# mlelarge/graph_neural_net

Hardware: AMD Instinct MI355X
Metric: graph-pairs/sec FGNN fwd+bwd, N=50 regular pairs (higher is better)
Workload: dtype f32

## Files before the change

### graph_neural_net_amd/_lib.py

```python
import ctypes as C
import os

import torch

_HERE = os.path.dirname(os.path.abspath(__file__))
LIB_PATH = os.environ.get('FGNN_LIB') or os.path.join(_HERE, 'libfgnn_hip.so')

FGNN_H = 32
FGNN_TILE = 32
FGNN_MAX_DEPTH = 3
FGNN_RANGE_WG = 256
FGNN_LSAP_MAX_N = 2048
FGNN_SCORE_SPLIT = 4

c_float_p = C.c_void_p


class Slab(C.Structure):
    _fields_ = [('ptr', C.c_void_p), ('gstride', C.c_longlong), ('ldp', C.c_longlong), ('C', C.c_int),
                ('nrm', C.c_void_p), ('beta', C.c_void_p)]


class MlpFwdArgs(C.Structure):
    _fields_ = [('G', C.c_int), ('N', C.c_int), ('depth', C.c_int), ('nmlp', C.c_int),
                ('nvalid', C.c_void_p),
                ('a', Slab), ('b', Slab),
                ('W', (C.c_void_p * FGNN_MAX_DEPTH) * 2),
                ('bias', (C.c_void_p * FGNN_MAX_DEPTH) * 2),
                ('z', C.c_void_p * 2),
                ('ldz', C.c_longlong),
                ('part', C.c_void_p * 2),
                ('cnt', C.c_void_p), ('packed', C.c_void_p), ('xbits', C.c_void_p), ('xdeg', C.c_void_p),
                ('ranges', C.c_void_p), ('cu_share', C.c_int)]


class DwJob(C.Structure):
    _fields_ = [('dy', C.c_void_p), ('d_gstride', C.c_longlong), ('d_ld', C.c_longlong), ('relu_mask', C.c_void_p),
                ('x', C.c_void_p), ('x_gstride', C.c_longlong), ('x_ld', C.c_longlong), ('M', C.c_int), ('K', C.c_int)]


class ChainLayer(C.Structure):
    _fields_ = [('W', C.c_void_p), ('w_ostride', C.c_longlong), ('w_kstride', C.c_longlong), ('bias', C.c_void_p),
                ('M', C.c_int), ('K', C.c_int), ('relu', C.c_int), ('mask', C.c_void_p), ('out', C.c_void_p),
                ('o_gstride', C.c_longlong)]


class ChainArgs(C.Structure):
    _fields_ = [('x', C.c_void_p), ('x_gstride', C.c_longlong), ('x_ld', C.c_longlong), ('depth', C.c_int),
                ('layer', ChainLayer * 3), ('o_ld', C.c_longlong), ('nvalid', C.c_void_p), ('G', C.c_int), ('N', C.c_int)]


class Mlp64Args(C.Structure):
    _fields_ = [('x', C.c_void_p), ('x_gstride', C.c_longlong), ('x_ld', C.c_longlong), ('cin', C.c_int),
                ('xb', C.c_void_p), ('xb_gstride', C.c_longlong), ('xb_ld', C.c_longlong), ('cb', C.c_int),
                ('packed', C.c_void_p), ('nvalid', C.c_void_p), ('G', C.c_int), ('N', C.c_int),
                ('out', C.c_void_p), ('o_gstride', C.c_longlong), ('o_ld', C.c_longlong),
                ('dz', C.c_void_p), ('dz_gstride', C.c_longlong), ('dz_ld', C.c_longlong),
                ('dx', C.c_void_p), ('dx_gstride', C.c_longlong), ('dx_ld', C.c_longlong),
                ('dxb', C.c_void_p), ('dxb_gstride', C.c_longlong), ('dxb_ld', C.c_longlong),
                ('accumulate_dx', C.c_int), ('accumulate_dxb', C.c_int),
                ('wpart', C.c_void_p)]


class Mlp64PackJob(C.Structure):
    _fields_ = [('W', C.c_void_p * 3), ('bias', C.c_void_p * 3), ('cin', C.c_int), ('packed', C.c_void_p)]


class MlpBwdArgs(C.Structure):
    _fields_ = [('G', C.c_int), ('N', C.c_int), ('depth', C.c_int),
                ('nvalid', C.c_void_p),
                ('a', Slab), ('b', Slab),
                ('W', C.c_void_p * FGNN_MAX_DEPTH),
                ('bias', C.c_void_p * FGNN_MAX_DEPTH),
                ('dy', C.c_void_p), ('dgstride', C.c_longlong), ('ldd', C.c_longlong),
                ('z', C.c_void_p), ('zgstride', C.c_longlong), ('ldz', C.c_longlong),
                ('coef', C.c_void_p), ('s12', C.c_void_p), ('znrm', C.c_void_p),
                ('dxa', C.c_void_p), ('dxa_gstride', C.c_longlong), ('dxa_ld', C.c_longlong),
                ('dxb', C.c_void_p), ('dxb_gstride', C.c_longlong), ('dxb_ld', C.c_longlong),
                ('accumulate_a', C.c_int), ('accumulate_b', C.c_int),
                ('wpart', C.c_void_p), ('s12part', C.c_void_p), ('packed', C.c_void_p),
                ('s12tiles', C.c_void_p), ('s12_out', C.c_void_p), ('xbits', C.c_void_p), ('xdeg', C.c_void_p),
                ('ranges', C.c_void_p), ('cu_share', C.c_int)]


class Slab16(C.Structure):
    _fields_ = [('ptr', C.c_void_p), ('gstride', C.c_longlong), ('ldp', C.c_longlong), ('C', C.c_int),
                ('nrm', C.c_void_p), ('beta', C.c_void_p)]


class MlpFwd16Args(C.Structure):
    _fields_ = [('G', C.c_int), ('N', C.c_int), ('ldr', C.c_int), ('depth', C.c_int), ('nmlp', C.c_int),
                ('nvalid', C.c_void_p),
                ('a', Slab16), ('b', Slab16),
                ('z', C.c_void_p * 2), ('ldz', C.c_longlong),
                ('part', C.c_void_p * 2), ('cnt', C.c_void_p), ('packed', C.c_void_p), ('ranges', C.c_void_p)]


class MlpBwd16Args(C.Structure):
    _fields_ = [('G', C.c_int), ('N', C.c_int), ('ldr', C.c_int), ('depth', C.c_int),
                ('nvalid', C.c_void_p),
                ('a', Slab16), ('b', Slab16),
                ('dy', C.c_void_p), ('dgstride', C.c_longlong), ('ldd', C.c_longlong),
                ('z', C.c_void_p), ('zgstride', C.c_longlong), ('ldz', C.c_longlong),
                ('coef', C.c_void_p),
                ('dxa', C.c_void_p), ('dxa_gstride', C.c_longlong), ('dxa_ld', C.c_longlong),
                ('dxb', C.c_void_p), ('dxb_gstride', C.c_longlong), ('dxb_ld', C.c_longlong),
                ('accumulate_a', C.c_int), ('accumulate_b', C.c_int),
                ('wpart', C.c_void_p), ('s12part', C.c_void_p), ('packed', C.c_void_p), ('ranges', C.c_void_p)]


class GradJob(C.Structure):
    _fields_ = [('wpart', C.c_void_p), ('count', C.c_int), ('out', C.c_void_p), ('s12', C.c_void_p),
                ('nrm', C.c_void_p), ('dgn_w', C.c_void_p), ('dgn_b', C.c_void_p), ('rows', C.c_int), ('scale', C.c_float), ('scale_dev', C.c_void_p)]


class PackJob(C.Structure):
    _fields_ = [('kind', C.c_int), ('ca', C.c_int), ('cb', C.c_int), ('depth', C.c_int), ('nmlp', C.c_int),
                ('W', (C.c_void_p * FGNN_MAX_DEPTH) * 2), ('bias', (C.c_void_p * FGNN_MAX_DEPTH) * 2),
                ('out', C.c_void_p)]


class PairgenArgs(C.Structure):
    _fields_ = [('seed', C.c_ulonglong), ('first', C.c_longlong), ('B', C.c_int), ('N', C.c_int),
                ('family', C.c_int), ('noise_model', C.c_int), ('edge_density', C.c_double),
                ('thr_edge', C.c_ulonglong), ('thr_noise1', C.c_ulonglong), ('thr_noise2', C.c_ulonglong),
                ('thr_vertex', C.c_ulonglong), ('swaps_per_edge', C.c_int),
                ('bits1', C.c_void_p), ('bits2', C.c_void_p), ('nvalid', C.c_void_p)]


MAX_GRAD_JOBS = 16
MAX_PACK_JOBS = 24
_VP, _LL, _I, _F = C.c_void_p, C.c_longlong, C.c_int, C.c_float

_SIGNATURES = {
    'fgnn_last_error': [],
    'fgnn_version': [],
    'fgnn_tiles_per_graph': [_I],
    'fgnn_mlp_bwd_num_workgroups': [],
    'fgnn_pack_floats': [_I, _I, _I, _I, _I],
    'fgnn_pack_operands': [_VP, _I, _VP],
    'fgnn_mlp_fwd': [C.POINTER(MlpFwdArgs), _VP],
    'fgnn_pack_x3_floats': [_I, _I, _I, _I, _I],
    'fgnn_pack_x3_operands': [_VP, _I, _VP],
    'fgnn_mlp_fwd_x3': [C.POINTER(MlpFwdArgs), _VP],
    'fgnn_debug_mlp_fwd_masks': [C.POINTER(MlpFwdArgs), _VP, _VP, _VP],
    'fgnn_debug_mlp_fwd_x3_masks': [C.POINTER(MlpFwdArgs), _VP, _VP, _VP],
    'fgnn_debug_matmul_variant': [_I],
    'fgnn_gn_finalize': [_VP, _VP, _VP, _VP, _I, _I, _I, _F, _VP, _VP],
    'fgnn_gn_finalize2': [_VP, _VP, _VP, _VP, _VP, _VP, _I, _I, _I, _F, _VP, _VP, _VP],
    'fgnn_gn_plane_supported': [_I],
    'fgnn_gn_plane_fwd': [_VP, _LL, _LL, _VP, _VP, _VP, _I, _I, _I, _F, _VP, _LL, _LL, _VP, _VP],
    'fgnn_gn_plane_bwd': [_VP, _LL, _LL, _VP, _LL, _LL, _VP, _VP, _I, _I, _I, _VP, _LL, _LL, _VP, _VP, _VP, _VP],
    'fgnn_gn_stats': [_VP, _LL, _LL, _VP, _VP, _I, _I, _I, _F, _VP, _VP],
    'fgnn_gn_apply': [_VP, _LL, _LL, _VP, _VP, _VP, _I, _I, _I, _VP, _LL, _LL, _VP],
    'fgnn_ragged_tile_ranges': [_VP, _I, _I, _VP, _VP],
    'fgnn_ragged_tile_ranges_order': [_VP, _I, _I, _VP, _VP, _VP],
    'fgnn_ragged_tile_ranges16': [_VP, _I, _I, _I, _VP, _VP],
    'fgnn_conv1x1_dw_multi': [C.POINTER(DwJob), _I, _VP, _I, _I, _VP, _VP],
    'fgnn_conv_chain_supported': [_I, _I, C.POINTER(C.c_int)],
    'fgnn_conv_chain': [C.POINTER(ChainArgs), _VP],
    'fgnn_mlp64_supported': [_I, _I, _I],
    'fgnn_mlp64_num_workgroups': [],
    'fgnn_mlp64_param_count': [_I],
    'fgnn_mlp64_packed_floats': [_I],
    'fgnn_mlp64_pack': [_VP, _VP, _VP, _VP, _VP, _VP, _I, _VP, _VP],
    'fgnn_mlp64_pack_multi': [C.POINTER(Mlp64PackJob), _I, _VP],
    'fgnn_mlp64_fwd': [C.POINTER(Mlp64Args), _VP],
    'fgnn_mlp64_bwd': [C.POINTER(Mlp64Args), _VP],
    'fgnn_conv1x1': [_VP, _LL, _LL, _VP, _VP, _LL, _LL, _VP, _I, _VP, _I, _I, _I, _I, _VP, _LL, _LL, _VP],
    'fgnn_conv1x1_dw_chunks': [_I, _I],
    'fgnn_conv1x1_dw': [_VP, _LL, _LL, _VP, _VP, _LL, _LL, _VP, _I, _I, _I, _I, _VP, _VP],
    'fgnn_chan_matmul_fwd': [C.POINTER(Slab), C.POINTER(Slab), _VP, _I, _I, _VP, _LL, _LL, _VP],
    'fgnn_chan_matmul_fwd_ord': [C.POINTER(Slab), C.POINTER(Slab), _VP, _I, _I, _VP, _LL, _LL, _VP, _I, _VP],
    'fgnn_chan_matmul_fwd_fin_supported': [_I],
    'fgnn_chan_matmul_fwd_fin': [C.POINTER(Slab), C.POINTER(Slab), _VP, _VP, _VP, _VP, _VP, _F, _VP, _I, _I, _VP, _LL, _LL, _VP],
    'fgnn_chan_matmul_fwd_fin_ord': [C.POINTER(Slab), C.POINTER(Slab), _VP, _VP, _VP, _VP, _VP, _F, _VP, _I, _I, _VP, _LL, _LL, _VP, _I, _VP],
    'fgnn_colmax_fwd': [C.POINTER(Slab), _VP, _I, _I, _VP, _VP, _VP],
    'fgnn_colmax_fwd_fin_supported': [_I],
    'fgnn_colmax_fwd_fin': [C.POINTER(Slab), _VP, _VP, _VP, _F, _VP, _I, _I, _VP, _VP, _VP],
    'fgnn_score_ce_fwd': [_VP, _VP, _VP, _I, _I, _I, _VP, _VP, _VP, _VP],
    'fgnn_score_row_blocks': [_I, _I],
    'fgnn_score_ce_fwd_blocks': [_VP, _VP, _VP, _I, _I, _I, _I, _VP, _VP, _VP, _VP],
    'fgnn_score_ce_bwd': [_VP, _VP, _VP, _VP, _VP, _VP, _I, _I, _I, _VP, _VP, _VP],
    'fgnn_inv_node_count': [_VP, _I, _VP, _VP],
    'fgnn_score_bwd': [_VP, _VP, _VP, _VP, _I, _I, _I, _VP, _VP, _VP],
    'fgnn_ce_fwd': [_VP, _VP, _I, _I, _VP, _VP, _VP],
    'fgnn_ce_bwd': [_VP, _VP, _VP, _VP, _I, _I, _VP, _VP],
    'fgnn_colmax_bwd': [_VP, _VP, _VP, _I, _I, _I, _VP, _LL, _LL, C.POINTER(Slab), _VP, _VP],
    'fgnn_gn_bwd_stats': [_VP, _LL, _LL, _VP, _LL, _LL, _VP, _VP, _I, _I, _I, _VP, _VP],
    'fgnn_gn_bwd_coef': [_VP, _VP, _VP, _I, _I, _I, _VP, _VP, _VP, _VP],
    'fgnn_gn_bwd_coef_tiles': [_VP, _VP, _VP, _I, _I, _I, _VP, _VP, _VP],
    'fgnn_grad_finalize': [_VP, _I, _I, _I, _I, _VP],
    'fgnn_gn_bwd_apply': [_VP, _LL, _LL, _VP, _LL, _LL, _VP, _VP, _I, _I, _I, _VP, _LL, _LL, _VP],
    'fgnn_mlp_bwd': [C.POINTER(MlpBwdArgs), _VP],
    'fgnn_mlp_bwd_x3': [C.POINTER(MlpBwdArgs), _VP],
    'fgnn_mlp_bwd_pair': [C.POINTER(MlpBwdArgs), C.POINTER(MlpBwdArgs), _VP],
    'fgnn_mlp_bwd_t16': [C.POINTER(MlpBwdArgs), _VP],
    'fgnn_mlp_bwd_t16_supported': [C.POINTER(MlpBwdArgs)],
    'fgnn_mlp_bwd_pair_t16': [C.POINTER(MlpBwdArgs), C.POINTER(MlpBwdArgs), _VP],
    'fgnn_mlp_bwd_pair_x3': [C.POINTER(MlpBwdArgs), C.POINTER(MlpBwdArgs), _VP],
    'fgnn_block1_struct_supported': [_I, _I, _I],
    'fgnn_block1_struct_table_floats': [_I],
    'fgnn_block1_struct_ws_floats': [_I, _I],
    'fgnn_block1_struct_rows': [_I, _I],
    'fgnn_block1_struct_fwd': [_VP, _VP, _I, _I, _VP, _VP, _VP, _VP, _VP, C.c_float, _VP, _VP, _VP, _LL, _LL, _VP, _VP, _VP, _VP, _VP, _VP, _VP],
    'fgnn_block1_struct_bwd': [_VP, _VP, _I, _I, _VP, _VP, _VP, _VP, _VP, _VP, _VP, _VP, _LL, _LL, _VP, _VP, _VP, _VP, _VP, _VP],
    'fgnn_block1_struct_fwd_pack': [_VP, _VP, _I, _I, _VP, _VP, _VP, _VP, _VP, C.c_float, _VP, _VP, _VP, _LL, _LL, _VP, _VP, _VP, _VP, _VP, _VP, _VP, _I, _VP],
    'fgnn_block1_struct_fwd16_pack': [_VP, _VP, _I, _I, _I, _VP, _VP, _VP, _VP, _VP, C.c_float, _VP, _VP, _VP, _LL, _LL, _VP, _VP, _VP, _VP, _VP, _VP, _VP, _I, _VP],
    'fgnn_block1_struct_fwd16': [_VP, _VP, _I, _I, _I, _VP, _VP, _VP, _VP, _VP, C.c_float, _VP, _VP, _VP, _LL, _LL, _VP, _VP, _VP, _VP, _VP, _VP, _VP],
    'fgnn_block1_struct_bwd16': [_VP, _VP, _I, _I, _I, _VP, _VP, _VP, _VP, _VP, _VP, _VP, _VP, _LL, _LL, _VP, _VP, _VP, _VP, _VP, _VP],
    'fgnn_mlp_bwd_coef_tiles_supported': [_I, _I],
    'fgnn_mlp_param_count': [_I, _I],
    'fgnn_reduce_partials': [_VP, _I, _I, _VP, _VP],
    'fgnn_chan_matmul_bwd': [C.POINTER(Slab), C.POINTER(Slab), _VP, _LL, _LL, _VP, _I, _I, _VP, _VP, _LL, _LL, _VP, _VP, _VP],
    'fgnn_chan_matmul_bwd_ord': [C.POINTER(Slab), C.POINTER(Slab), _VP, _LL, _LL, _VP, _I, _I, _VP, _VP, _LL, _LL, _VP, _VP, _VP, _I, _VP],
    'fgnn_sum_scale': [_VP, _I, _I, _F, _VP, _VP],
    'fgnn_adam_step': [_VP, _VP, _VP, _VP, _I, C.c_double, C.c_double, C.c_double, C.c_double, _I, C.c_double, _VP],
    'fgnn_adam_step_dev': [_VP, _VP, _VP, _VP, _I, _VP, _VP, _VP],
    'fgnn_expand_adjacency': [_VP, _VP, _I, _I, _VP, _VP],
    'fgnn_pack_adjacency': [_VP, _VP, _I, _I, _VP, _VP, _VP],
    'fgnn_pack_adjacency_ld': [_VP, _VP, _I, _I, _I, _VP, _VP, _VP],
    'fgnn_pack_adjacency_pair': [_VP, _VP, _VP, _VP, _I, _I, _I, _VP, _VP, _VP, _VP, _VP],
    'fgnn_adjacency_degree': [_VP, _VP, _I, _I, _VP, _VP],
    'fgnn_accuracy_max': [_VP, _VP, _I, _I, _VP, _VP],
    'fgnn_lsap_accuracy': [_VP, _LL, _I, _VP, _I, _I, _VP, _VP, _VP],
    'fgnn_pairgen_supported': [_I, _I, _I],
    'fgnn_pairgen': [C.POINTER(PairgenArgs), _VP],
    'fgnn_tiles_per_graph16': [_I, _I],
    'fgnn_to_bf16': [_VP, _VP, _I, _I, _I, _I, _VP, _LL, _LL, _VP],
    'fgnn_from_bf16': [_VP, _LL, _LL, _I, _I, _I, _I, _VP, _VP],
    'fgnn_pack16_floats': [_I, _I, _I, _I, _I],
    'fgnn_pack16_operands': [_VP, _I, _VP],
    'fgnn_mlp_fwd16': [C.POINTER(MlpFwd16Args), _VP],
    'fgnn_debug_mlp_fwd16_masks': [C.POINTER(MlpFwd16Args), _VP, _VP, _VP],
    'fgnn_gn_finalize_tpg': [_VP, _VP, _VP, _VP, _I, _I, _I, _I, _F, _VP, _VP],
    'fgnn_gn_finalize2_tpg': [_VP, _VP, _VP, _VP, _VP, _VP, _I, _I, _I, _I, _F, _VP, _VP, _VP],
    'fgnn_gn_bwd_coef_tiles_tpg': [_VP, _VP, _VP, _I, _I, _I, _I, _VP, _VP, _VP],
    'fgnn_chan_matmul_fwd16': [C.POINTER(Slab16), C.POINTER(Slab16), _VP, _I, _I, _I, _VP, _LL, _LL, _VP],
    'fgnn_chan_matmul_fwd16_fin': [C.POINTER(Slab16), C.POINTER(Slab16), _VP, _VP, _VP, _VP, _VP, _F, _I, _VP, _I, _I, _I, _VP, _LL,
                                   _LL, _VP],
    'fgnn_chan_matmul_bwd16': [C.POINTER(Slab16), C.POINTER(Slab16), _VP, _LL, _LL, _VP, _I, _I, _I, _VP, _VP, _LL, _LL, _VP, _VP, _VP],
    'fgnn_chan_matmul_bwd16_t': [C.POINTER(Slab16), C.POINTER(Slab16), _VP, _LL, _LL, _VP, _I, _VP, _I, _I, _I, _VP, _VP, _LL, _LL,
                                 _VP, _VP, _VP],
    'fgnn_chan_matmul_bwd16_tc': [C.POINTER(Slab16), C.POINTER(Slab16), _VP, _LL, _LL, _VP, _I, _VP, _I, _I, _I, _VP, _VP, _LL, _LL,
                                  _VP, _VP, _VP, _VP, _VP],
    'fgnn_colmax_bwd16_coef': [_VP, _VP, _VP, _I, _I, _I, _I, _VP, _LL, _LL, C.POINTER(Slab16), _VP, _VP, _VP],
    'fgnn_colmax_fwd16': [C.POINTER(Slab16), _VP, _I, _I, _I, _VP, _VP, _VP],
    'fgnn_colmax_bwd16': [_VP, _VP, _VP, _I, _I, _I, _I, _VP, _LL, _LL, C.POINTER(Slab16), _VP, _VP],
    'fgnn_mlp_bwd16': [C.POINTER(MlpBwd16Args), _VP],
    'fgnn_mlp_bwd16_pair': [C.POINTER(MlpBwd16Args), C.POINTER(MlpBwd16Args), _VP],
}
_RESTYPES = {'fgnn_last_error': C.c_char_p, 'fgnn_block1_struct_ws_floats': C.c_longlong}
EXPORTS = tuple(_SIGNATURES)

_lib = None


def load():
    global _lib
    if _lib is not None:
        return _lib
    if not os.path.exists(LIB_PATH):
        raise RuntimeError(
            'graph_neural_net_amd: %s is missing. Build it with '
            '`python -c "import __graft_entry__ as g; g.build()"` or `make -C graph_neural_net_amd/csrc`. '
            'There is no CPU fallback.' % LIB_PATH)
    lib = C.CDLL(LIB_PATH)
    for name, argtypes in _SIGNATURES.items():
        fn = getattr(lib, name)
        fn.argtypes = argtypes
        fn.restype = _RESTYPES.get(name, C.c_int)
# ... 73 lines not shown
```

### graph_neural_net_amd/csrc/mlp_bwd.hip

```cpp
#include "fgnn_common.h"
#include "fgnn_pack.h"

#ifdef FGNN_PHASES
__device__ unsigned long long *g_phase_buf = nullptr;
__device__ int g_phase_sel = 0;
#define PH_DECL unsigned long long ph_[16] = {0, 0, 0, 0, 0, 0, 0, 0, 0, 0, 0, 0, 0, 0, 0, 0}; unsigned long long ph_last_ = __builtin_amdgcn_s_memtime();
#define PH(k) { const unsigned long long t_ = __builtin_amdgcn_s_memtime(); ph_[k] += t_ - ph_last_; ph_last_ = t_; }
#define PH_FLUSH if (g_phase_buf && g_phase_sel == CA * 100 + CB && (threadIdx.x & 63) == 0) { for (int k_ = 0; k_ < 16; ++k_) g_phase_buf[((long long)blockIdx.x * NW + wv) * 16 + k_] = ph_[k_]; }
#else
#define PH_DECL
#define PH(k) __builtin_amdgcn_sched_barrier(0);
#define PH_FLUSH
#endif

namespace {

constexpr int TLD = 36;
constexpr int TILE_F = 32 * TLD;
constexpr int BWD_WG = 256;

struct TileCtx {
    int g, tt, p, i, jj;
    bool inb;
};
// ... 628 lines not shown
    static_assert(PCOUNT % 4 == 0, "partials are summed four at a time");
    float4 *out = reinterpret_cast<float4 *>(A.wpart + (long long)blockIdx.x * PCOUNT);
    const float4 *part4 = reinterpret_cast<const float4 *>(smem);
    for (int e = threadIdx.x; e < PCOUNT / 4; e += 64 * NW) {
        float4 a = part4[e];
#pragma unroll
        for (int w = 1; w < NW; ++w) {
            const float4 b = part4[w * (PCOUNT / 4) + e];
            a.x += b.x;
            a.y += b.y;
            a.z += b.z;
            a.w += b.w;
        }
        out[e] = a;
    }
    PH(11)
    PH_FLUSH
}

template <int CA, int CB, int DEPTH, bool PK = false, bool SKIP = false>
int launch_bwd_impl(const fgnn_mlp_bwd_args *a, int tpg, int total, hipStream_t st) {
    constexpr int LDS = BwdLayout<CA, CB, DEPTH>::LDS_F * 4;
    static_assert(LDS <= 160 * 1024, "LDS budget");
    static LdsAttrCache attr_cache;
    (void)fgnn_raise_lds(attr_cache, (const void *)mlp_bwd_kernel<CA, CB, DEPTH, PK, SKIP>, LDS);
    hipLaunchKernelGGL((mlp_bwd_kernel<CA, CB, DEPTH, PK, SKIP>), dim3(a->cu_share == 2 && !SKIP ? BWD_WG / 2 : BWD_WG), dim3(64 * NW), LDS, st,
                       *a, tpg, total);
    FGNN_LAUNCH_CHECK();
    return 0;
}
template <int CA, int CB, int DEPTH, bool PK = false>
int launch_bwd(const fgnn_mlp_bwd_args *a, int tpg, int total, hipStream_t st) {
    static_assert(BWD_WG == FGNN_RANGE_WG, "fgnn_ragged_tile_ranges splits for the backward grid");
    if (a->ranges) return launch_bwd_impl<CA, CB, DEPTH, PK, true>(a, tpg, total, st);
    return launch_bwd_impl<CA, CB, DEPTH, PK, false>(a, tpg, total, st);
}

template <int DEPTH>
int dispatch_c(const fgnn_mlp_bwd_args *a, int tpg, int total, hipStream_t st) {
    const int ca = a->a.C, cb = a->b.C;
    if (a->xbits) {
        if constexpr (DEPTH == 3) {
            if (ca == 2 && cb == 0) return launch_bwd<2, 0, DEPTH, true>(a, tpg, total, st);
            if (ca == 32 && cb == 2) return launch_bwd<32, 2, DEPTH, true>(a, tpg, total, st);
        }
        fgnn_set_error("fgnn_mlp_bwd: xbits needs depth 3 and a 2-channel slab (2 or 32+2 input channels), got depth %d, %d + %d",
                       DEPTH, ca, cb);
        return 1;
    }
#define FGNN_CASE(A_, B_) \
    if (ca == A_ && cb == B_) return launch_bwd<A_, B_, DEPTH>(a, tpg, total, st);
    FGNN_CASE(2, 0)
    FGNN_CASE(16, 0)
    FGNN_CASE(32, 0)
    FGNN_CASE(32, 2)
    FGNN_CASE(32, 32)
#undef FGNN_CASE
    fgnn_set_error("fgnn_mlp_bwd: unsupported input channels (%d + %d); built for 2, 16, 32, 32+2, 32+32", ca, cb);
    return 1;
}

}

#ifdef FGNN_PHASES
extern "C" int fgnn_debug_phase_buffer(void *p, int ca, int cb) {
    const int sel = ca * 100 + cb;
    if (hipMemcpyToSymbol(HIP_SYMBOL(g_phase_sel), &sel, sizeof(sel)) != hipSuccess) return 1;
    return hipMemcpyToSymbol(HIP_SYMBOL(g_phase_buf), &p, sizeof(p)) == hipSuccess ? 0 : 1;
}
#endif

extern "C" int fgnn_mlp_bwd_num_workgroups(void) { return BWD_WG; }

extern "C" int fgnn_mlp_bwd_coef_tiles_supported(int G, int N) {
    const long long tpg = fgnn_tiles_per_graph(N), total = (long long)G * tpg;
    const long long per_wg = (total + BWD_WG - 1) / BWD_WG;
    return (per_wg + tpg - 2) / tpg + 1 <= FGNN_BWD_COEF_GRAPHS ? 1 : 0;
}

extern "C" int fgnn_mlp_param_count(int Cin, int depth) { return 32 * Cin + 32 + (depth - 1) * (32 * 32 + 32); }

extern "C" int fgnn_mlp_bwd(const fgnn_mlp_bwd_args *a, void *stream) {
    FGNN_CHECK(a != nullptr, "fgnn_mlp_bwd: null args");
    FGNN_CHECK(a->G > 0 && a->N > 0, "fgnn_mlp_bwd: bad G=%d N=%d", a->G, a->N);
    FGNN_CHECK(a->depth >= 1 && a->depth <= FGNN_MAX_DEPTH, "fgnn_mlp_bwd: depth %d not in 1..%d", a->depth, FGNN_MAX_DEPTH);
    const bool pk_a = a->xbits && a->a.C == 2, pk_b = a->xbits && a->b.C == 2;
    FGNN_CHECK((a->a.ptr || pk_a) && a->a.C > 0, "fgnn_mlp_bwd: slab a missing");
    FGNN_CHECK(a->b.C == 0 || a->b.ptr || pk_b, "fgnn_mlp_bwd: slab b has channels but no pointer");
    FGNN_CHECK(!a->xbits || a->xdeg, "fgnn_mlp_bwd: xbits without xdeg (fgnn_adjacency_degree)");
    FGNN_CHECK(!(pk_a && a->dxa) && !(pk_b && a->dxb), "fgnn_mlp_bwd: no gradient with respect to the packed adjacency");
    FGNN_CHECK(a->dy && a->z && a->wpart, "fgnn_mlp_bwd: missing dy/z/wpart");
    FGNN_CHECK(a->coef || (a->s12 && a->znrm) || (a->s12tiles && a->znrm), "fgnn_mlp_bwd: need coef, or s12 + znrm, or s12tiles + znrm");
    {
        const long long lim = 0x7fffffffll / 4, G = a->G;
        FGNN_CHECK(G * a->a.gstride < lim && G * a->b.gstride < lim && G * a->dgstride < lim && G * a->zgstride < lim &&
                   G * a->dxa_gstride < lim && G * a->dxb_gstride < lim,
                   "fgnn_mlp_bwd: a tensor exceeds 2 GiB (32-bit buffer addressing); split the batch");
    }
    for (int l = 0; l < a->depth; ++l) FGNN_CHECK(a->W[l] && a->bias[l], "fgnn_mlp_bwd: missing weights layer %d", l);
    const int tpg = fgnn_tiles_per_graph(a->N);
    const long long total = (long long)a->G * tpg;
    FGNN_CHECK(total < (1ll << 30), "fgnn_mlp_bwd: too many tiles");
    FGNN_CHECK(!a->ranges || (a->nvalid && !a->s12tiles), "fgnn_mlp_bwd: ranges need nvalid and exclude s12tiles");
    FGNN_CHECK(!a->s12tiles || a->b.C > 0, "fgnn_mlp_bwd: s12tiles is built into the two-slab kernels only; use fgnn_gn_bwd_coef_tiles");
    FGNN_CHECK(!a->s12tiles || fgnn_mlp_bwd_coef_tiles_supported(a->G, a->N),
               "fgnn_mlp_bwd: s12tiles needs a workgroup's tile range to span <= %d graphs (G=%d N=%d); "
               "use fgnn_gn_bwd_coef_tiles", FGNN_BWD_COEF_GRAPHS, a->G, a->N);
    hipStream_t st = (hipStream_t)stream;
    if (a->depth == 1) return dispatch_c<1>(a, tpg, (int)total, st);
    if (a->depth == 2) return dispatch_c<2>(a, tpg, (int)total, st);
    return dispatch_c<3>(a, tpg, (int)total, st);
}
```

### graph_neural_net_amd/csrc/mlp_bwd_pair.hip

```cpp
#include "fgnn_tile.h"
#include "fgnn_pack.h"

namespace {

constexpr int BWD_WG = 256;
constexpr int NW = 8;
constexpr int NP = 4;

DEVI float4 coef_from_sums(const float4 n, const float2 sv, float nv) {
    const float m = nv * nv;
    float4 k;
    k.x = n.x;
    k.y = n.y;
    k.z = m > 0.f ? -n.y * sv.y * n.w / m : 0.f;
    k.w = m > 0.f ? -n.y * sv.x / m : 0.f;
    return k;
}
DEVI float4 coef_record(const fgnn_mlp_bwd_args &A, int g, int ch) {
    if (A.coef) return reinterpret_cast<const float4 *>(A.coef)[(long long)g * FGNN_H + ch];
    const float4 n = reinterpret_cast<const float4 *>(A.znrm)[(long long)g * FGNN_H + ch];
    const float2 sv = reinterpret_cast<const float2 *>(A.s12)[(long long)g * FGNN_H + ch];
    return coef_from_sums(n, sv, (float)nvalid_of(A.nvalid, g, A.N));
}

// ... 360 lines not shown
        }
    }

    constexpr int PCOUNT = L::PCOUNT;
#pragma unroll
    for (int l = 0; l < DEPTH; ++l) db[l] += __shfl_xor(db[l], 32);
    if constexpr (VW0) {
#pragma unroll
        for (int r = 0; r < 32; ++r) w0v[r] = half_sum(w0v[r]);
#pragma unroll
        for (int r = 0; r < 16; ++r) b0v[r] = half_sum(b0v[r]);
    }
    __syncthreads();
    {
        float *red = smem + wv * PCOUNT;
#pragma unroll
        for (int r = 0; r < 16; ++r) {
            const int o = ch_of(r, h);
            if constexpr (VW0) {
                if (j == 0) {
                    red[o * CA] = w0v[2 * r];
                    red[o * CA + 1] = w0v[2 * r + 1];
                    red[32 * CA + o] = b0v[r];
                }
            } else {
                if (j < CA) red[o * CA + j] = dW0a[r];
            }
        }
        int off = 32 * CA;
#pragma unroll
        for (int l = 0; l < DEPTH; ++l) {
            if (l > 0) {
#pragma unroll
                for (int r = 0; r < 16; ++r) red[off + ch_of(r, h) * 32 + j] = dWh[l - 1][r];
                off += 1024;
            }
            if (h == 0 && !(VW0 && l == 0)) red[off + j] = db[l];
            off += 32;
        }
    }
    __syncthreads();
    static_assert(PCOUNT % 4 == 0, "partials are summed four at a time");
    const float4 *part4 = reinterpret_cast<const float4 *>(smem);
    for (int e = threadIdx.x; e < 2 * (PCOUNT / 4); e += 64 * NW) {
        const int m = e >= PCOUNT / 4 ? 1 : 0, ee = e - m * (PCOUNT / 4);
        float4 a = part4[(4 * m) * (PCOUNT / 4) + ee];
#pragma unroll
        for (int w = 1; w < NP; ++w) {
            const float4 b = part4[(4 * m + w) * (PCOUNT / 4) + ee];
            a.x += b.x;
            a.y += b.y;
            a.z += b.z;
            a.w += b.w;
        }
        reinterpret_cast<float4 *>(P.m[m].wpart + (long long)blockIdx.x * PCOUNT)[ee] = a;
    }
}

template <int CA, bool PK, bool SKIP>
int launch_pair_impl(const fgnn_mlp_bwd_args *a1, const fgnn_mlp_bwd_args *a2, int tpg, int total, hipStream_t st) {
    constexpr int LDS = PairLayout<CA>::LDS_F * 4;
    static_assert(LDS <= 160 * 1024, "LDS budget");
    static LdsAttrCache attr_cache;
    (void)fgnn_raise_lds(attr_cache, (const void *)mlp_bwd_pair_kernel<CA, PK, SKIP>, LDS);
    PairArgs P;
    P.m[0] = *a1;
    P.m[1] = *a2;
    hipLaunchKernelGGL((mlp_bwd_pair_kernel<CA, PK, SKIP>), dim3(a1->cu_share == 2 && !SKIP ? BWD_WG / 2 : BWD_WG), dim3(64 * NW), LDS, st, P,
                       tpg, total);
    FGNN_LAUNCH_CHECK();
    return 0;
}
template <int CA, bool PK>
int launch_pair(const fgnn_mlp_bwd_args *a1, const fgnn_mlp_bwd_args *a2, int tpg, int total, hipStream_t st) {
    static_assert(BWD_WG == FGNN_RANGE_WG, "fgnn_ragged_tile_ranges splits for the backward grid");
    if (a1->ranges) return launch_pair_impl<CA, PK, true>(a1, a2, tpg, total, st);
    return launch_pair_impl<CA, PK, false>(a1, a2, tpg, total, st);
}

}

extern "C" int fgnn_mlp_bwd_pair(const fgnn_mlp_bwd_args *a1, const fgnn_mlp_bwd_args *a2, void *stream) {
    FGNN_CHECK(a1 && a2, "fgnn_mlp_bwd_pair: null args");
    FGNN_CHECK(BWD_WG == fgnn_mlp_bwd_num_workgroups(), "fgnn_mlp_bwd_pair: workgroup count differs from fgnn_mlp_bwd");
    FGNN_CHECK(a1->G > 0 && a1->N > 0 && a1->G == a2->G && a1->N == a2->N && a1->depth == a2->depth,
               "fgnn_mlp_bwd_pair: the two MLPs must share G, N and depth");
    FGNN_CHECK(mlp_bwd_pair_supported(a1->a.C, a1->depth) && a1->b.C == 0 && a2->b.C == 0,
               "fgnn_mlp_bwd_pair: built for depth 3 and ONE input slab of 2 or 32 channels (got depth %d, %d + %d); use fgnn_mlp_bwd",
               a1->depth, a1->a.C, a1->b.C);
    FGNN_CHECK(a1->a.ptr == a2->a.ptr && a1->a.C == a2->a.C && a1->a.gstride == a2->a.gstride && a1->a.ldp == a2->a.ldp &&
               a1->a.nrm == a2->a.nrm && a1->a.beta == a2->a.beta && a1->xbits == a2->xbits && a1->xdeg == a2->xdeg &&
               a1->nvalid == a2->nvalid, "fgnn_mlp_bwd_pair: the two MLPs must read the same input slab");
    FGNN_CHECK(a1->ranges == a2->ranges && (!a1->ranges || a1->nvalid), "fgnn_mlp_bwd_pair: both MLPs take the same ranges (with nvalid)");
    FGNN_CHECK(a1->packed && a2->packed, "fgnn_mlp_bwd_pair: needs both operand images (fgnn_pack_operands, kind 1)");
    FGNN_CHECK(!a1->dxa && !a1->s12part, "fgnn_mlp_bwd_pair: the input gradient and its tile sums belong to the SECOND argument block");
    FGNN_CHECK(!a1->s12tiles && !a2->s12tiles, "fgnn_mlp_bwd_pair: s12tiles is an mlp3 feature");
    const bool pk_a = a1->xbits && a1->a.C == 2;
    FGNN_CHECK((a1->a.ptr || pk_a), "fgnn_mlp_bwd_pair: slab a missing");
    FGNN_CHECK(!a1->xbits || a1->xdeg, "fgnn_mlp_bwd_pair: xbits without xdeg (fgnn_adjacency_degree)");
    FGNN_CHECK(!(a2->dxa && a2->a.C != 32), "fgnn_mlp_bwd_pair: the input gradient exists for the 32-channel slab only; use fgnn_mlp_bwd");
    for (const fgnn_mlp_bwd_args *a : {a1, a2}) {
        FGNN_CHECK(a->dy && a->z && a->wpart, "fgnn_mlp_bwd_pair: missing dy/z/wpart");
        FGNN_CHECK(a->coef || (a->s12 && a->znrm), "fgnn_mlp_bwd_pair: need coef, or s12 + znrm");
        const long long lim = 0x7fffffffll / 4, G = a->G;
        FGNN_CHECK(G * a->a.gstride < lim && G * a->dgstride < lim && G * a->zgstride < lim && G * a->dxa_gstride < lim,
                   "fgnn_mlp_bwd_pair: a tensor exceeds 2 GiB (32-bit buffer addressing); split the batch");
    }
    const int tpg = fgnn_tiles_per_graph(a1->N);
    const long long total = (long long)a1->G * tpg;
    FGNN_CHECK(total < (1ll << 30), "fgnn_mlp_bwd_pair: too many tiles");
    hipStream_t st = (hipStream_t)stream;
    if (a1->xbits) return launch_pair<2, true>(a1, a2, tpg, (int)total, st);
    if (a1->a.C == 2) return launch_pair<2, false>(a1, a2, tpg, (int)total, st);
    return launch_pair<32, false>(a1, a2, tpg, (int)total, st);
}
```

### graph_neural_net_amd/csrc/mlp_bwd_pair_t16.hip

```cpp
#include "fgnn_t16.h"
#include "fgnn_pack.h"

#ifdef FGNN_PHASES
__device__ unsigned long long *g_phase16_buf = nullptr;
#define PH_DECL unsigned long long ph_[16] = {0, 0, 0, 0, 0, 0, 0, 0, 0, 0, 0, 0, 0, 0, 0, 0}; unsigned long long ph_last_ = __builtin_amdgcn_s_memtime();
#define PH(k) { const unsigned long long t_ = __builtin_amdgcn_s_memtime(); ph_[k] += t_ - ph_last_; ph_last_ = t_; }
#define PH_FLUSH if (g_phase16_buf && (threadIdx.x & 63) == 0) { for (int k_ = 0; k_ < 16; ++k_) g_phase16_buf[((long long)blockIdx.x * NW + wv) * 16 + k_] = ph_[k_]; }
#else
#define PH_DECL
#define PH(k)
#define PH_FLUSH
#endif

namespace {

using namespace t16;

constexpr int BWD_WG = 256;
constexpr int NW = 8;
constexpr int NP = 4;

DEVI float4 coef_from_sums(const float4 n, const float2 sv, float nv) {
    const float m = nv * nv;
    float4 k;
// ... 336 lines not shown
    if constexpr (SKIP) {
        if (emit) {
            for (int t = T0 + pair; t < T1; t += NP) {
                const int g = t / tpg, tt = t - g * tpg;
                if (tile_live(tt, A.N, A.nvalid[g])) continue;
                if (lane < 32) reinterpret_cast<float2 *>(P.m[1].s12part)[((long long)g * tpg + tt) * FGNN_H + lane] = make_float2(0.f, 0.f);
            }
        }
    }

    constexpr int PCOUNT = L::PCOUNT;
#pragma unroll
    for (int b = 0; b < 2; ++b) {
        db0[b] += __shfl_xor(db0[b], 16);
        db0[b] += __shfl_xor(db0[b], 32);
        db1[b] += __shfl_xor(db1[b], 16);
        db1[b] += __shfl_xor(db1[b], 32);
        db2[b] += __shfl_xor(db2[b], 16);
        db2[b] += __shfl_xor(db2[b], 32);
    }
    __syncthreads();
    PH(10)
    {
        float *red = smem + wv * PCOUNT;
        auto put = [&](int off, const f32x4 (&dW)[4], const float (&db)[2]) {
#pragma unroll
            for (int mb = 0; mb < 2; ++mb)
#pragma unroll
                for (int nb = 0; nb < 2; ++nb)
#pragma unroll
                    for (int r = 0; r < 4; ++r) red[off + row_chan(16 * mb + 4 * q + r) * 32 + row_chan(16 * nb + px)] = dW[2 * mb + nb][r];
            if (q == 0) {
                red[off + 1024 + row_chan(px)] = db[0];
                red[off + 1024 + row_chan(16 + px)] = db[1];
            }
        };
        put(0, dW0, db0);
        put(1056, dW1, db1);
        put(2112, dW2, db2);
    }
    __syncthreads();
    static_assert(PCOUNT % 4 == 0 && PCOUNT == 3 * 1056, "partials are summed four at a time");
    const float4 *part4 = reinterpret_cast<const float4 *>(smem);
    for (int e = threadIdx.x; e < 2 * (PCOUNT / 4); e += 64 * NW) {
        const int m = e >= PCOUNT / 4 ? 1 : 0, ee = e - m * (PCOUNT / 4);
        float4 a = part4[(4 * m) * (PCOUNT / 4) + ee];
#pragma unroll
        for (int w = 1; w < NP; ++w) {
            const float4 b = part4[(4 * m + w) * (PCOUNT / 4) + ee];
            a.x += b.x;
            a.y += b.y;
            a.z += b.z;
            a.w += b.w;
        }
        reinterpret_cast<float4 *>(P.m[m].wpart + (long long)blockIdx.x * PCOUNT)[ee] = a;
    }
    PH(11)
    PH_FLUSH
}

template <bool SKIP, bool HAS_DX>
int launch_pair16(const fgnn_mlp_bwd_args *a1, const fgnn_mlp_bwd_args *a2, int tpg, int total, hipStream_t st) {
    constexpr int LDS = PairLayout16::LDS_F * 4;
    static_assert(LDS <= 160 * 1024, "LDS budget");
    static LdsAttrCache attr_cache;
    (void)fgnn_raise_lds(attr_cache, (const void *)mlp_bwd_pair_t16_kernel<SKIP, HAS_DX>, LDS);
    PairArgs P;
    P.m[0] = *a1;
    P.m[1] = *a2;
    hipLaunchKernelGGL((mlp_bwd_pair_t16_kernel<SKIP, HAS_DX>), dim3(a1->cu_share == 2 && !SKIP ? BWD_WG / 2 : BWD_WG), dim3(64 * NW), LDS, st, P, tpg,
                       total);
    FGNN_LAUNCH_CHECK();
    return 0;
}

}

#ifdef FGNN_PHASES
extern "C" int fgnn_debug_phase_buffer_t16(void *p) { return hipMemcpyToSymbol(HIP_SYMBOL(g_phase16_buf), &p, sizeof(p)) == hipSuccess ? 0 : 1; }
#endif

extern "C" int fgnn_mlp_bwd_pair_t16(const fgnn_mlp_bwd_args *a1, const fgnn_mlp_bwd_args *a2, void *stream) {
    FGNN_CHECK(a1 && a2, "fgnn_mlp_bwd_pair_t16: null args");
    FGNN_CHECK(BWD_WG == fgnn_mlp_bwd_num_workgroups() && BWD_WG == FGNN_RANGE_WG, "fgnn_mlp_bwd_pair_t16: workgroup count differs from fgnn_mlp_bwd");
    FGNN_CHECK(a1->G > 0 && a1->N > 0 && a1->G == a2->G && a1->N == a2->N && a1->depth == a2->depth,
               "fgnn_mlp_bwd_pair_t16: the two MLPs must share G, N and depth");
    FGNN_CHECK(a1->depth == 3 && a1->a.C == 32 && a1->b.C == 0 && a2->b.C == 0 && !a1->xbits && !a2->xbits,
               "fgnn_mlp_bwd_pair_t16: built for depth 3 and ONE dense input slab of 32 channels (got depth %d, %d + %d); use fgnn_mlp_bwd_pair",
               a1->depth, a1->a.C, a1->b.C);
    FGNN_CHECK(a1->a.ptr && a1->a.ptr == a2->a.ptr && a1->a.C == a2->a.C && a1->a.gstride == a2->a.gstride && a1->a.ldp == a2->a.ldp &&
               a1->a.nrm == a2->a.nrm && a1->a.beta == a2->a.beta && a1->nvalid == a2->nvalid,
               "fgnn_mlp_bwd_pair_t16: the two MLPs must read the same input slab");
    FGNN_CHECK(a1->ranges == a2->ranges && (!a1->ranges || a1->nvalid), "fgnn_mlp_bwd_pair_t16: both MLPs take the same ranges (with nvalid)");
    FGNN_CHECK(a1->packed && a2->packed, "fgnn_mlp_bwd_pair_t16: needs both operand images (fgnn_pack_operands, kind 5)");
    FGNN_CHECK(!a1->dxa && !a1->s12part, "fgnn_mlp_bwd_pair_t16: the input gradient and its tile sums belong to the SECOND argument block");
    FGNN_CHECK(!a1->s12tiles && !a2->s12tiles, "fgnn_mlp_bwd_pair_t16: s12tiles is an mlp3 feature");
    FGNN_CHECK(a1->N <= 256, "fgnn_mlp_bwd_pair_t16: N <= 256 (division-free pixel decode)");
    for (const fgnn_mlp_bwd_args *a : {a1, a2}) {
        FGNN_CHECK(a->dy && a->z && a->wpart, "fgnn_mlp_bwd_pair_t16: missing dy/z/wpart");
        FGNN_CHECK(a->coef || (a->s12 && a->znrm), "fgnn_mlp_bwd_pair_t16: need coef, or s12 + znrm");
        const long long lim = 0x7fffffffll / 4, G = a->G;
        FGNN_CHECK(G * a->a.gstride < lim && G * a->dgstride < lim && G * a->zgstride < lim && G * a->dxa_gstride < lim,
                   "fgnn_mlp_bwd_pair_t16: a tensor exceeds 2 GiB (32-bit buffer addressing); split the batch");
    }
    const int tpg = fgnn_tiles_per_graph(a1->N);
    const long long total = (long long)a1->G * tpg;
    FGNN_CHECK(total < (1ll << 29), "fgnn_mlp_bwd_pair_t16: too many tiles");
    hipStream_t st = (hipStream_t)stream;
    if (a2->dxa) return a1->ranges ? launch_pair16<true, true>(a1, a2, tpg, (int)total, st) : launch_pair16<false, true>(a1, a2, tpg, (int)total, st);
    return a1->ranges ? launch_pair16<true, false>(a1, a2, tpg, (int)total, st) : launch_pair16<false, false>(a1, a2, tpg, (int)total, st);
}
```

### graph_neural_net_amd/csrc/mlp_bwd_pair_x3.hip

```cpp
#include "fgnn_tile.h"
#include "fgnn_pack.h"
#include "fgnn_x3.h"

namespace {

#ifdef FGNN_PHASES
__device__ unsigned long long *g_px3_phase_buf = nullptr;
#define PH_DECL unsigned long long ph_[16] = {0, 0, 0, 0, 0, 0, 0, 0, 0, 0, 0, 0, 0, 0, 0, 0}; unsigned long long ph_last_ = __builtin_amdgcn_s_memtime();
#define PH(k) { const unsigned long long t_ = __builtin_amdgcn_s_memtime(); ph_[k] += t_ - ph_last_; ph_last_ = t_; }
#define PH_FLUSH if (g_px3_phase_buf && CA == 32 && (threadIdx.x & 63) == 0) { for (int k_ = 0; k_ < 16; ++k_) g_px3_phase_buf[((long long)blockIdx.x * NW + wv) * 16 + k_] = ph_[k_]; }
#else
#define PH_DECL
#define PH(k)
#define PH_FLUSH
#endif

constexpr int BWD_WG = 256;
constexpr int NW = 8;
constexpr int NP = 4;

DEVI float4 coef_from_sums(const float4 n, const float2 sv, float nv) {
    const float m = nv * nv;
    float4 k;
    k.x = n.x;
// ... 359 lines not shown
        prev_tile = tile;
        PH(8)
    }

    constexpr int PCOUNT = L::PCOUNT;
    float db[DEPTH];
#pragma unroll
    for (int l = 0; l < DEPTH; ++l) {
        db[l] = -ndb[l];
        db[l] += __shfl_xor(db[l], 32);
    }
    f32x16 dWh[2];
#pragma unroll
    for (int r = 0; r < 16; ++r) {
        dWh[0][r] = PARK[r * 64 + lane];
        dWh[1][r] = PARK[1024 + r * 64 + lane];
    }
    PH(12)
    __syncthreads();
    PH(10)
    {
        float *red = smem + wv * PCOUNT;
#pragma unroll
        for (int r = 0; r < 16; ++r) {
            const int o = ch_of(r, h);
            if (j < CA) red[o * CA + j] = dW0a[r];
        }
        int off = 32 * CA;
#pragma unroll
        for (int l = 0; l < DEPTH; ++l) {
            if (l > 0) {
#pragma unroll
                for (int r = 0; r < 16; ++r) red[off + ch_of(r, h) * 32 + j] = dWh[l - 1][r];
                off += 1024;
            }
            if (h == 0) red[off + j] = db[l];
            off += 32;
        }
    }
    __syncthreads();
    static_assert(PCOUNT % 4 == 0, "partials are summed four at a time");
    const float4 *part4 = reinterpret_cast<const float4 *>(smem);
    for (int e = threadIdx.x; e < 2 * (PCOUNT / 4); e += 64 * NW) {
        const int m = e >= PCOUNT / 4 ? 1 : 0, ee = e - m * (PCOUNT / 4);
        float4 a = part4[(4 * m) * (PCOUNT / 4) + ee];
#pragma unroll
        for (int w = 1; w < NP; ++w) {
            const float4 b = part4[(4 * m + w) * (PCOUNT / 4) + ee];
            a.x += b.x;
            a.y += b.y;
            a.z += b.z;
            a.w += b.w;
        }
        reinterpret_cast<float4 *>(P.m[m].wpart + (long long)blockIdx.x * PCOUNT)[ee] = a;
    }
    PH(11)
    PH_FLUSH
}

template <int CA, bool PK>
int launch_pair_x3(const fgnn_mlp_bwd_args *a1, const fgnn_mlp_bwd_args *a2, int tpg, int total, hipStream_t st) {
    constexpr int LDS = PairX3Layout<CA>::LDS_F * 4;
    static_assert(LDS <= 160 * 1024, "LDS budget");
    static LdsAttrCache attr_cache;
    (void)fgnn_raise_lds(attr_cache, (const void *)mlp_bwd_pair_x3_kernel<CA, PK>, LDS);
    PairArgs P;
    P.m[0] = *a1;
    P.m[1] = *a2;
    hipLaunchKernelGGL((mlp_bwd_pair_x3_kernel<CA, PK>), dim3(a1->cu_share == 2 ? BWD_WG / 2 : BWD_WG), dim3(64 * NW), LDS, st, P, tpg, total);
    FGNN_LAUNCH_CHECK();
    return 0;
}

}

#ifdef FGNN_PHASES
extern "C" int fgnn_debug_phase_buffer_px3(void *p) {
    return hipMemcpyToSymbol(HIP_SYMBOL(g_px3_phase_buf), &p, sizeof(p)) == hipSuccess ? 0 : 1;
}
#endif

extern "C" int fgnn_mlp_bwd_pair_x3(const fgnn_mlp_bwd_args *a1, const fgnn_mlp_bwd_args *a2, void *stream) {
    FGNN_CHECK(a1 && a2, "fgnn_mlp_bwd_pair_x3: null args");
    FGNN_CHECK(BWD_WG == fgnn_mlp_bwd_num_workgroups(), "fgnn_mlp_bwd_pair_x3: workgroup count differs from fgnn_mlp_bwd");
    FGNN_CHECK(a1->G > 0 && a1->N > 0 && a1->G == a2->G && a1->N == a2->N && a1->depth == a2->depth,
               "fgnn_mlp_bwd_pair_x3: the two MLPs must share G, N and depth");
    FGNN_CHECK(mlp_bwd_pair_supported(a1->a.C, a1->depth) && a1->b.C == 0 && a2->b.C == 0,
               "fgnn_mlp_bwd_pair_x3: built for depth 3 and ONE input slab of 2 or 32 channels (got depth %d, %d + %d); use fgnn_mlp_bwd",
               a1->depth, a1->a.C, a1->b.C);
    FGNN_CHECK(a1->a.ptr == a2->a.ptr && a1->a.C == a2->a.C && a1->a.gstride == a2->a.gstride && a1->a.ldp == a2->a.ldp &&
               a1->a.nrm == a2->a.nrm && a1->a.beta == a2->a.beta && a1->xbits == a2->xbits && a1->xdeg == a2->xdeg &&
               a1->nvalid == a2->nvalid, "fgnn_mlp_bwd_pair_x3: the two MLPs must read the same input slab");
    FGNN_CHECK(!a1->ranges && !a2->ranges, "fgnn_mlp_bwd_pair_x3: no padding-tile skipping (ranges); use fgnn_mlp_bwd_pair for ragged batches");
    FGNN_CHECK(a1->packed && a2->packed, "fgnn_mlp_bwd_pair_x3: needs both operand images (fgnn_pack_x3_operands, kind 1)");
    FGNN_CHECK(!a1->dxa && !a1->s12part, "fgnn_mlp_bwd_pair_x3: the input gradient and its tile sums belong to the SECOND argument block");
    FGNN_CHECK(!a1->s12tiles && !a2->s12tiles, "fgnn_mlp_bwd_pair_x3: s12tiles is an mlp3 feature");
    const bool pk_a = a1->xbits && a1->a.C == 2;
    FGNN_CHECK((a1->a.ptr || pk_a), "fgnn_mlp_bwd_pair_x3: slab a missing");
    FGNN_CHECK(!a1->xbits || a1->xdeg, "fgnn_mlp_bwd_pair_x3: xbits without xdeg (fgnn_adjacency_degree)");
    FGNN_CHECK(!(a2->dxa && a2->a.C != 32), "fgnn_mlp_bwd_pair_x3: the input gradient exists for the 32-channel slab only; use fgnn_mlp_bwd");
    FGNN_CHECK(a1->ldd == a1->ldz && a2->ldd == a1->ldd && a2->ldz == a1->ldd && (!a2->dxa || a2->dxa_ld == a1->ldd) &&
               (a1->a.C != 32 || a1->a.ldp == a1->ldd),
               "fgnn_mlp_bwd_pair_x3: dy, z, d_in (and a 32-channel input slab) must share one channel stride");
    for (const fgnn_mlp_bwd_args *a : {a1, a2}) {
        FGNN_CHECK(a->dy && a->z && a->wpart, "fgnn_mlp_bwd_pair_x3: missing dy/z/wpart");
        FGNN_CHECK(a->coef || (a->s12 && a->znrm), "fgnn_mlp_bwd_pair_x3: need coef, or s12 + znrm");
        const long long lim = 0x7fffffffll / 4, G = a->G;
        FGNN_CHECK(G * a->a.gstride < lim && G * a->dgstride < lim && G * a->zgstride < lim && G * a->dxa_gstride < lim,
                   "fgnn_mlp_bwd_pair_x3: a tensor exceeds 2 GiB (32-bit buffer addressing); split the batch");
    }
    const int tpg = fgnn_tiles_per_graph(a1->N);
    const long long total = (long long)a1->G * tpg;
    FGNN_CHECK(total < (1ll << 30), "fgnn_mlp_bwd_pair_x3: too many tiles");
    hipStream_t st = (hipStream_t)stream;
    if (a1->xbits) return launch_pair_x3<2, true>(a1, a2, tpg, (int)total, st);
    if (a1->a.C == 2) return launch_pair_x3<2, false>(a1, a2, tpg, (int)total, st);
    return launch_pair_x3<32, false>(a1, a2, tpg, (int)total, st);
}
```

### graph_neural_net_amd/csrc/mlp_bwd_t16.hip

```cpp
#include "fgnn_t16.h"
#include "fgnn_pack.h"

namespace {

using namespace t16;

constexpr int BWD_WG = 256;
constexpr int NW = 8;

DEVI float4 coef_from_sums(const float4 n, const float2 sv, float nv) {
    const float m = nv * nv;
    float4 k;
    k.x = n.x;
    k.y = n.y;
    k.z = m > 0.f ? -n.y * sv.y * n.w / m : 0.f;
    k.w = m > 0.f ? -n.y * sv.x / m : 0.f;
    return k;
}
DEVI int graph_nv(const rsrc_t &rnv, bool ragged, int g, int N) {
    const int v = __builtin_amdgcn_raw_buffer_load_b32(rnv, g * 4, 0, 0);
    return __builtin_amdgcn_readfirstlane(ragged ? v : N);
}

template <int CB>
struct Layout16 {
    static constexpr int DEPTH = 3;
    static constexpr PkBwd PK = pk_bwd(32, CB, DEPTH);
    static constexpr int OFF_W0A = PK.off_w1a, OFF_W0B = PK.off_w1b, OFF_W1 = PK.off_wh, OFF_WT1 = PK.off_wt, OFF_WT2 = PK.off_wt + 16;
    static constexpr int OFF_WT0A = PK.off_wt0a, OFF_WT0B = PK.off_wt0b;
    static constexpr int BIAS_F = PK.bias_f;
    static constexpr int WEIGHT_F = pk_pad_floats(PK.floats);
    static constexpr int NSLOT = 5;
    static constexpr int CIN = 32 + CB;
    static constexpr int PCOUNT = 32 * CIN + 32 + (DEPTH - 1) * (32 * 32 + 32);
    static constexpr int TILE_OFF = WEIGHT_F;
    static constexpr int REC_OFF = TILE_OFF + NW * NSLOT * TILE_F;
    static constexpr int WGK_OFF = REC_OFF + NW * 256;
    static constexpr int LIVE_OFF = WGK_OFF + FGNN_BWD_COEF_GRAPHS * 128;
    static constexpr int MAIN_F = LIVE_OFF + LIVE_LIST_CAP + NW;
    static constexpr int RED_F = NW * PCOUNT;
    static constexpr int LDS_F = MAIN_F > RED_F ? MAIN_F : RED_F;
};

template <int CB, bool PKD, bool SKIP, bool DXB>
__global__ __launch_bounds__(64 * NW, 2) void mlp_bwd_t16_kernel(const fgnn_mlp_bwd_args A, const int tpg, const int total_tiles) {
    extern __shared__ __attribute__((aligned(16))) float smem[];
    using L = Layout16<CB>;
    constexpr bool NB = CB == 32;
    const int lane = threadIdx.x & 63, wv = __builtin_amdgcn_readfirstlane(threadIdx.x >> 6);
    const int px = lane & 15, q = lane >> 4;
    const int P2 = A.N * A.N, hpg = 2 * tpg;
    const View va = make_view(A.a.ptr, A.a.gstride, A.a.ldp, A.G);
    const View vb = make_view(A.b.ptr, A.b.gstride, A.b.ldp, A.G);
    PackedSrc ps = {};
    if constexpr (PKD) ps = make_packed_src(A.xbits, A.xdeg, A.G, A.N);
    const View vdy = make_view(A.dy, A.dgstride, A.ldd, A.G);
    const View vz = make_view(A.z, A.zgstride, A.ldz, A.G);
    const View vdxa = make_view(A.dxa, A.dxa_gstride, A.dxa_ld, A.G);
    const View vdxb = make_view(A.dxb, A.dxb_gstride, A.dxb_ld, A.G);

    float *wl = smem;
    float *my = smem + L::TILE_OFF + wv * (L::NSLOT * TILE_F);
    float *XA = my, *XB = my + TILE_F, *S0 = my + 2 * TILE_F, *S1 = my + 3 * TILE_F, *S2 = my + 4 * TILE_F;
    const int lane_base = tile_lane_base(px, q);

    f32x4 dW0a[4], dW0b[4], dW1[4], dW2[4];
    float db0[2] = {0.f, 0.f}, db1[2] = {0.f, 0.f}, db2[2] = {0.f, 0.f}, dbx[2] = {0.f, 0.f};
#pragma unroll
    for (int k = 0; k < 4; ++k) dW0a[k] = dW0b[k] = dW1[k] = dW2[k] = zero4();

    const int nwg = gridDim.x;
    const int qq = total_tiles / nwg, rem = total_tiles % nwg;
    int T0 = blockIdx.x * qq + ((int)blockIdx.x < rem ? (int)blockIdx.x : rem);
    int T1 = T0 + qq + ((int)blockIdx.x < rem ? 1 : 0);
    if constexpr (SKIP) {
        T0 = A.ranges[blockIdx.x];
        T1 = A.ranges[blockIdx.x + 1];
    }
    const int H0 = 2 * T0, H1 = 2 * T1;
    const bool ragged = A.nvalid != nullptr;
    const rsrc_t rnv = __builtin_amdgcn_make_buffer_rsrc(const_cast<int *>(A.nvalid), 0, ragged ? A.G * 4 : 0, 0x00020000);
    const float rcpN = 1.f / (float)A.N;
    const bool from_tiles = A.s12tiles != nullptr;
    const int g0 = T0 / tpg;
    float4 *wgK = reinterpret_cast<float4 *>(smem + L::WGK_OFF);

    int live_cnt = 0;
    int *live_list = reinterpret_cast<int *>(smem + L::LIVE_OFF);
    int nlive = 0, lk = wv - NW;
    bool use_list = false;
    if constexpr (SKIP) {
        nlive = build_live_list(live_list, live_list + LIVE_LIST_CAP, T0, T1, tpg, FGNN_TILE, A.N, A.nvalid, threadIdx.x, 64 * NW);
        use_list = nlive <= LIVE_LIST_CAP;
    }
    auto next_half = [&](int h) {
        if constexpr (SKIP) {
            if (use_list) {
                int r = H1;
                while (true) {
                    lk += NW;
                    if ((lk >> 1) >= nlive) break;
                    const int t = live_list[lk >> 1], g = t / tpg, hh = 2 * (t - g * tpg) + (lk & 1);
                    if (hh * 16 < P2) {
                        r = 2 * t + (lk & 1);
                        break;
                    }
                }
                return __builtin_amdgcn_readfirstlane(r);
            }
            while (h < H1) {
                const int g = h / hpg, hh = h - g * hpg;
                const int nv = A.nvalid[g];
                if (hh * 16 < P2 && tile_live(hh >> 1, A.N, nv)) {
                    const bool mine = live_cnt % NW == wv;
                    ++live_cnt;
                    if (mine) break;
                    ++h;
                } else if ((hh >> 1) * FGNN_TILE / A.N >= nv) {
                    h = (g + 1) * hpg;
                } else {
                    ++h;
                }
            }
            return __builtin_amdgcn_readfirstlane(h < H1 ? h : H1);
        } else {
            while (h < H1) {
                const int g = h / hpg, hh = h - g * hpg;
                if (hh * 16 < P2) break;
                h += NW;
            }
            return __builtin_amdgcn_readfirstlane(h);
        }
    };

    pk_glds<NW>(smem, A.packed, L::WEIGHT_F, wv, lane);

    float mean[8], av[8], beta[8], kx[8], ky[8], kz[8], kw[8];
#pragma unroll
    for (int s = 0; s < 8; ++s) {
        mean[s] = 0.f;
        av[s] = 1.f;
        beta[s] = (NB && A.b.nrm && A.b.beta) ? A.b.beta[chan_s(s) + chan_q(q)] : 0.f;
        kx[s] = ky[s] = kz[s] = kw[s] = 0.f;
    }
    float4 *rec = reinterpret_cast<float4 *>(smem + L::REC_OFF) + wv * 64;
    auto fetch_records = [&](int g, int nv) {
        if (lane < 32) {
            float4 k4;
            if (from_tiles) k4 = wgK[(g - g0) * 32 + lane];
            else if (A.coef) k4 = reinterpret_cast<const float4 *>(A.coef)[(long long)g * FGNN_H + lane];
            else {
                const float4 n = reinterpret_cast<const float4 *>(A.znrm)[(long long)g * FGNN_H + lane];
                const float2 sv = reinterpret_cast<const float2 *>(A.s12)[(long long)g * FGNN_H + lane];
                k4 = coef_from_sums(n, sv, (float)nv);
            }
            rec[lane] = k4;
            if (NB && A.b.nrm) rec[32 + lane] = reinterpret_cast<const float4 *>(A.b.nrm)[(long long)g * A.b.C + lane];
        }
    };
    auto read_records = [&]() {
#pragma unroll
        for (int s = 0; s < 8; ++s) {
            const float4 k4 = rec[chan_s(s) + chan_q(q)];
            kx[s] = k4.x;
            ky[s] = k4.y;
            kz[s] = k4.z;
            kw[s] = k4.w;
            if (NB && A.b.nrm) {
                const float4 n = rec[32 + chan_s(s) + chan_q(q)];
                mean[s] = n.x;
                av[s] = n.y;
            }
        }
    };

    constexpr int NXB = CB == 32 ? 8 : 1;
    float xa[8], xb[NXB], dyr[8], zr[8];
    auto load_x = [&](int h) {
        const bool act = h < H1;
        const int g = __builtin_amdgcn_readfirstlane(act ? h / hpg : 0);
        const int p = (act ? h - g * hpg : 0) * 16 + px;
        const bool inb = act && p < P2;
        load8(xa, va, lane_voff(va, q, p, inb), g * va.gs4);
        if constexpr (CB == 32) {
            load8(xb, vb, lane_voff(vb, q, p, inb), g * vb.gs4);
        } else if constexpr (PKD) {
            int i, jj;
            row_col(p, A.N, rcpN, i, jj);
            const int ob = (inb && q == 0) ? (i * ps.words + (jj >> 5)) * 4 : OOB_OFF;
            const int od = (inb && q == 1 && i == jj) ? i * 4 : OOB_OFF;
            const unsigned w = (unsigned)__builtin_amdgcn_raw_buffer_load_b32(ps.bits, ob, g * ps.N * ps.words * 4, 0);
            const float d = __builtin_bit_cast(float, __builtin_amdgcn_raw_buffer_load_b32(ps.deg, od, g * ps.N * 4, 0));
            xb[0] = q == 0 ? (((w >> (jj & 31)) & 1u) ? 1.f : 0.f) : d;
        } else {
            xb[0] = buf_load(vb, (inb && q < 2) ? q * vb.ld4 + 4 * p : OOB_OFF, g * vb.gs4);
        }
    };
    auto load_dyz = [&](int h) {
        const bool act = h < H1;
        const int g = __builtin_amdgcn_readfirstlane(act ? h / hpg : 0);
        const int p = (act ? h - g * hpg : 0) * 16 + px;
        const bool inb = act && p < P2;
        load8(dyr, vdy, lane_voff(vdy, q, p, inb), g * vdy.gs4);
        load8(zr, vz, lane_voff(vz, q, p, inb), g * vz.gs4);
    };

    int h = next_half(SKIP ? H0 : H0 + wv);
    load_x(h);
    int cached_g = -1, cur_nv = A.N;

    if (from_tiles) {
        const int g1 = T1 > T0 ? (T1 - 1) / tpg : g0 - 1;
        float2 *scr = reinterpret_cast<float2 *>(smem + L::TILE_OFF);
        const int cc = threadIdx.x & 31, sl = threadIdx.x >> 5;
        for (int g = g0; g <= g1; ++g) {
            float p1 = 0.f, p2 = 0.f;
            constexpr int TS = (64 * NW) / 32, U = 8;
            for (int t0 = sl; t0 < tpg; t0 += TS * U) {
                float2 v[U];
#pragma unroll
                for (int k = 0; k < U; ++k) {
                    const int t = t0 + TS * k;
                    v[k] = reinterpret_cast<const float2 *>(A.s12tiles)[((long long)g * tpg + (t < tpg ? t : 0)) * FGNN_H + cc];
                }
#pragma unroll
                for (int k = 0; k < U; ++k) {
                    if (t0 + TS * k < tpg) {
                        p1 += v[k].x;
                        p2 += v[k].y;
                    }
                }
            }
            scr[sl * 32 + cc] = make_float2(p1, p2);
            __syncthreads();
            if (threadIdx.x < 32) {
                float s1 = 0.f, s2 = 0.f;
#pragma unroll
                for (int k = 0; k < (64 * NW) / 32; ++k) {
                    s1 += scr[k * 32 + cc].x;
                    s2 += scr[k * 32 + cc].y;
                }
                const float2 sv = make_float2(s1, s2);
                if (A.s12_out) reinterpret_cast<float2 *>(A.s12_out)[(long long)g * FGNN_H + cc] = sv;
                const float4 n = reinterpret_cast<const float4 *>(A.znrm)[(long long)g * FGNN_H + cc];
                wgK[(g - g0) * 32 + cc] = coef_from_sums(n, sv, (float)graph_nv(rnv, ragged, g, A.N));
            }
            __syncthreads();
        }
    }
    if (h < H1) {
        const int g = h / hpg;
        cur_nv = graph_nv(rnv, ragged, g, A.N);
        fetch_records(g, cur_nv);
        cached_g = g;
    }
    if constexpr (CB == 2) {
        for (int e = lane; e < 16 * TLD; e += 64) XB[e] = 0.f;
    }
    __syncthreads();
    load_dyz(h);
    if (cached_g >= 0) read_records();

    while (h < H1) {
        const int hn = next_half(SKIP ? h + 1 : h + NW);
        const int g = __builtin_amdgcn_readfirstlane(h / hpg), hh = h - g * hpg;
        const int p = hh * 16 + px;
        const bool inb = p < P2;
        if (g != cached_g) {
            cur_nv = graph_nv(rnv, ragged, g, A.N);
            fetch_records(g, cur_nv);
            read_records();
            cached_g = g;
        }
        bool valid = inb;
        if (ragged) {
            int i, jj;
            row_col(p, A.N, rcpN, i, jj);
            valid = inb && i < cur_nv && jj < cur_nv;
        }
        const bool full = __ballot(valid) == ~0ull;

        float h1[8], h2[8];
        {
            float yb[NXB];
            if constexpr (NB) {
#pragma unroll
                for (int s = 0; s < 8; ++s) yb[s] = (xb[s] - mean[s]) * av[s] + beta[s];
            } else {
                yb[0] = xb[0];
            }
            stage8(XA, lane_base, xa);
            if constexpr (CB == 32) {
                stage8(XB, lane_base, yb);
            } else {
                if (q < 2) XB[8 * q * TLD + px] = yb[0];
            }
            f32x4 acc[2];
            load_bias(acc, wl + L::BIAS_F, 0, q);
            gemm32<L::OFF_W0A>(acc, wl, xa, lane);
            if constexpr (CB == 32) gemm32<L::OFF_W0B>(acc, wl, yb, lane);
            else gemm2<L::OFF_W0B>(acc, wl, q < 2 ? yb[0] : 0.f, lane);
            load_x(hn);
#pragma unroll
            for (int s = 0; s < 8; ++s) h1[s] = relu1(acc[s >> 2][s & 3]);
            stage8(S0, lane_base, h1);
            load_bias(acc, wl + L::BIAS_F, 1, q);
            gemm32<L::OFF_W1>(acc, wl, h1, lane);
#pragma unroll
            for (int s = 0; s < 8; ++s) h2[s] = relu1(acc[s >> 2][s & 3]);
            stage8(S1, lane_base, h2);
        }
        float dpre[8];
#pragma unroll
        for (int s = 0; s < 8; ++s) dpre[s] = fmaf(kz[s], zr[s] - kx[s], fmaf(ky[s], dyr[s], kw[s]));
        if (!full) {
#pragma unroll
            for (int s = 0; s < 8; ++s) dpre[s] = valid ? dpre[s] : 0.f;
        }
        stage8(S2, lane_base, dpre);
        load_dyz(hn);
        __builtin_amdgcn_sched_barrier(0);
        {
            f32x4 a2[2];
            a2[0] = a2[1] = zero4();
            gemm32<L::OFF_WT2>(a2, wl, dpre, lane);
            wgrad16(dW2, db2, S2, S1, lane);
#pragma unroll
            for (int s = 0; s < 8; ++s) dpre[s] = h2[s] > 0.f ? a2[s >> 2][s & 3] : 0.f;
        }
        __builtin_amdgcn_sched_barrier(0);
        stage8(S1, lane_base, dpre);
        {
            f32x4 a2[2];
            a2[0] = a2[1] = zero4();
            gemm32<L::OFF_WT1>(a2, wl, dpre, lane);
            wgrad16(dW1, db1, S1, S0, lane);
#pragma unroll
            for (int s = 0; s < 8; ++s) dpre[s] = h1[s] > 0.f ? a2[s >> 2][s & 3] : 0.f;
        }
        __builtin_amdgcn_sched_barrier(0);
        stage8(S2, lane_base, dpre);
        __builtin_amdgcn_sched_barrier(0);
        {
            f32x4 dx[2];
            float v[8];
            dx[0] = dx[1] = zero4();
            gemm32<L::OFF_WT0A>(dx, wl, dpre, lane);
            wgrad16(dW0a, db0, S2, XA, lane);
#pragma unroll
            for (int s = 0; s < 8; ++s) v[s] = dx[s >> 2][s & 3];
            store8(v, vdxa, lane_voff(vdxa, q, p, inb), g * vdxa.gs4);
            if constexpr (DXB) {
                dx[0] = dx[1] = zero4();
                gemm32<L::OFF_WT0B>(dx, wl, dpre, lane);
            }
            if constexpr (CB == 32) {
                wgrad16(dW0b, dbx, S2, XB, lane);
            } else {
                const int i = lane & 15;
                const float4 a0 = *reinterpret_cast<const float4 *>(S2 + i * TLD + 4 * q);
                const float4 a1 = *reinterpret_cast<const float4 *>(S2 + (16 + i) * TLD + 4 * q);
                const float4 b0 = *reinterpret_cast<const float4 *>(XB + i * TLD + 4 * q);
                dW0b[0] = mfma16(a0.x, b0.x, dW0b[0]);
                dW0b[2] = mfma16(a1.x, b0.x, dW0b[2]);
                dW0b[0] = mfma16(a0.y, b0.y, dW0b[0]);
                dW0b[2] = mfma16(a1.y, b0.y, dW0b[2]);
                dW0b[0] = mfma16(a0.z, b0.z, dW0b[0]);
                dW0b[2] = mfma16(a1.z, b0.z, dW0b[2]);
                dW0b[0] = mfma16(a0.w, b0.w, dW0b[0]);
                dW0b[2] = mfma16(a1.w, b0.w, dW0b[2]);
            }
            if constexpr (DXB) {
#pragma unroll
                for (int s = 0; s < 8; ++s) v[s] = dx[s >> 2][s & 3];
                store8(v, vdxb, lane_voff(vdxb, q, p, inb), g * vdxb.gs4);
            }
        }
        h = hn;
    }

    constexpr int PCOUNT = L::PCOUNT, CIN = L::CIN;
#pragma unroll
    for (int b = 0; b < 2; ++b) {
        db0[b] += __shfl_xor(db0[b], 16);
        db0[b] += __shfl_xor(db0[b], 32);
        db1[b] += __shfl_xor(db1[b], 16);
        db1[b] += __shfl_xor(db1[b], 32);
        db2[b] += __shfl_xor(db2[b], 16);
        db2[b] += __shfl_xor(db2[b], 32);
    }
    (void)dbx;
    __syncthreads();
    {
        float *red = smem + wv * PCOUNT;
#pragma unroll
        for (int mb = 0; mb < 2; ++mb)
#pragma unroll
            for (int nb = 0; nb < 2; ++nb)
#pragma unroll
                for (int r = 0; r < 4; ++r) {
                    const int o = row_chan(16 * mb + 4 * q + r), c = row_chan(16 * nb + px);
                    red[o * CIN + c] = dW0a[2 * mb + nb][r];
                    if (c < CB) red[o * CIN + 32 + c] = dW0b[2 * mb + nb][r];
                    red[32 * CIN + 32 + o * 32 + c] = dW1[2 * mb + nb][r];
                    red[32 * CIN + 32 + 1056 + o * 32 + c] = dW2[2 * mb + nb][r];
                }
        if (q == 0) {
            const int c0 = row_chan(px), c1 = row_chan(16 + px);
            red[32 * CIN + c0] = db0[0];
            red[32 * CIN + c1] = db0[1];
            red[32 * CIN + 32 + 1024 + c0] = db1[0];
            red[32 * CIN + 32 + 1024 + c1] = db1[1];
            red[32 * CIN + 32 + 1056 + 1024 + c0] = db2[0];
            red[32 * CIN + 32 + 1056 + 1024 + c1] = db2[1];
        }
    }
    __syncthreads();
    static_assert(PCOUNT % 4 == 0, "partials are summed four at a time");
    float4 *out = reinterpret_cast<float4 *>(A.wpart + (long long)blockIdx.x * PCOUNT);
    const float4 *part4 = reinterpret_cast<const float4 *>(smem);
    for (int e = threadIdx.x; e < PCOUNT / 4; e += 64 * NW) {
        float4 a = part4[e];
#pragma unroll
        for (int w = 1; w < NW; ++w) {
            const float4 b = part4[w * (PCOUNT / 4) + e];
            a.x += b.x;
            a.y += b.y;
            a.z += b.z;
            a.w += b.w;
        }
        out[e] = a;
    }
}

template <int CB, bool PKD, bool SKIP, bool DXB>
int launch16(const fgnn_mlp_bwd_args *a, int tpg, int total, hipStream_t st) {
    constexpr int LDS = Layout16<CB>::LDS_F * 4;
    static_assert(LDS <= 160 * 1024, "LDS budget");
    static LdsAttrCache attr_cache;
    (void)fgnn_raise_lds(attr_cache, (const void *)mlp_bwd_t16_kernel<CB, PKD, SKIP, DXB>, LDS);
    hipLaunchKernelGGL((mlp_bwd_t16_kernel<CB, PKD, SKIP, DXB>), dim3(a->cu_share == 2 && !SKIP ? BWD_WG / 2 : BWD_WG), dim3(64 * NW), LDS, st, *a,
                       tpg, total);
    FGNN_LAUNCH_CHECK();
    return 0;
}
template <int CB, bool PKD, bool DXB>
int launch16s(const fgnn_mlp_bwd_args *a, int tpg, int total, hipStream_t st) {
    return a->ranges ? launch16<CB, PKD, true, DXB>(a, tpg, total, st) : launch16<CB, PKD, false, DXB>(a, tpg, total, st);
}

}

extern "C" int fgnn_mlp_bwd_t16_supported(const fgnn_mlp_bwd_args *a) {
    if (!a || a->depth != 3 || a->a.C != 32 || a->a.nrm || !a->dxa || a->accumulate_a || a->accumulate_b || !a->packed || a->N > 256) return 0;
    if (a->b.C == 32) return (a->b.nrm && a->dxb && !a->xbits) ? 1 : 0;
    if (a->b.C == 2) return (!a->b.nrm && !a->dxb) ? 1 : 0;
    return 0;
}

extern "C" int fgnn_mlp_bwd_t16(const fgnn_mlp_bwd_args *a, void *stream) {
    FGNN_CHECK(a != nullptr, "fgnn_mlp_bwd_t16: null args");
    FGNN_CHECK(fgnn_mlp_bwd_t16_supported(a), "fgnn_mlp_bwd_t16: built for depth 3, slab a = 32 raw channels with dx stored, slab b = 32 normalised "
               "channels with dx stored or 2 raw channels without dx, an operand image of kind 5, N <= 256; use fgnn_mlp_bwd");
    FGNN_CHECK(a->G > 0 && a->N > 0 && a->a.ptr && (a->b.ptr || (a->xbits && a->b.C == 2)), "fgnn_mlp_bwd_t16: bad G / N / slabs");
    FGNN_CHECK(!a->xbits || a->xdeg, "fgnn_mlp_bwd_t16: xbits without xdeg (fgnn_adjacency_degree)");
    FGNN_CHECK(a->dy && a->z && a->wpart, "fgnn_mlp_bwd_t16: missing dy/z/wpart");
    FGNN_CHECK(a->coef || (a->s12 && a->znrm) || (a->s12tiles && a->znrm), "fgnn_mlp_bwd_t16: need coef, or s12 + znrm, or s12tiles + znrm");
    FGNN_CHECK(BWD_WG == fgnn_mlp_bwd_num_workgroups() && BWD_WG == FGNN_RANGE_WG, "fgnn_mlp_bwd_t16: workgroup count differs from fgnn_mlp_bwd");
    {
        const long long lim = 0x7fffffffll / 4, G = a->G;
        FGNN_CHECK(G * a->a.gstride < lim && G * a->b.gstride < lim && G * a->dgstride < lim && G * a->zgstride < lim &&
                   G * a->dxa_gstride < lim && G * a->dxb_gstride < lim,
                   "fgnn_mlp_bwd_t16: a tensor exceeds 2 GiB (32-bit buffer addressing); split the batch");
    }
    for (int l = 0; l < a->depth; ++l) FGNN_CHECK(a->W[l] && a->bias[l], "fgnn_mlp_bwd_t16: missing weights layer %d", l);
    const int tpg = fgnn_tiles_per_graph(a->N);
    const long long total = (long long)a->G * tpg;
    FGNN_CHECK(total < (1ll << 29), "fgnn_mlp_bwd_t16: too many tiles");
    FGNN_CHECK(!a->ranges || (a->nvalid && !a->s12tiles), "fgnn_mlp_bwd_t16: ranges need nvalid and exclude s12tiles");
    FGNN_CHECK(!a->s12tiles || fgnn_mlp_bwd_coef_tiles_supported(a->G, a->N), "fgnn_mlp_bwd_t16: s12tiles needs a workgroup's tile range to span <= %d graphs",
               FGNN_BWD_COEF_GRAPHS);
    hipStream_t st = (hipStream_t)stream;
    if (a->b.C == 32) return launch16s<32, false, true>(a, tpg, (int)total, st);
    if (a->xbits) return launch16s<2, true, false>(a, tpg, (int)total, st);
    return launch16s<2, false, false>(a, tpg, (int)total, st);
}
```

### graph_neural_net_amd/csrc/mlp_bwd_x3.hip

```cpp
#include "fgnn_tile.h"
#include "fgnn_pack.h"
#include "fgnn_x3.h"

namespace {

constexpr int BWD_WG = 256;

DEVI float4 coef_from_sums(const float4 n, const float2 sv, float nv) {
    const float m = nv * nv;
    float4 k;
    k.x = n.x;
    k.y = n.y;
    k.z = m > 0.f ? -n.y * sv.y * n.w / m : 0.f;
    k.w = m > 0.f ? -n.y * sv.x / m : 0.f;
    return k;
}
DEVI float4 coef_record(const fgnn_mlp_bwd_args &A, int g, int ch) {
    if (A.coef) return reinterpret_cast<const float4 *>(A.coef)[(long long)g * FGNN_H + ch];
    const float4 n = reinterpret_cast<const float4 *>(A.znrm)[(long long)g * FGNN_H + ch];
    const float2 sv = reinterpret_cast<const float2 *>(A.s12)[(long long)g * FGNN_H + ch];
    return coef_from_sums(n, sv, (float)nvalid_of(A.nvalid, g, A.N));
}

template <int CA, int CB, int NWT>
// ... 423 lines not shown
                }
#pragma unroll
                for (int r = 0; r < 16; ++r) buf_store(vb2[r], vdxb, voff, s0 + ((r & 3) + 8 * (r >> 2)) * vdxb.ld4);
            }
        }
        if constexpr (CA == 32 && CB == 0) {
#pragma unroll
            for (int s = 0; s < SA; ++s) xa[s] = nxa[s];
        }
    }

    constexpr int PCOUNT = L::PCOUNT;
#pragma unroll
    for (int l = 0; l < DEPTH; ++l) db[l] += __shfl_xor(db[l], 32);
    if constexpr (VW0) {
#pragma unroll
        for (int r = 0; r < 32; ++r) w0v[r] = half_sum(w0v[r]);
#pragma unroll
        for (int r = 0; r < 16; ++r) b0v[r] = half_sum(b0v[r]);
    }
    __syncthreads();
    {
        float *red = smem + wv * PCOUNT;
#pragma unroll
        for (int r = 0; r < 16; ++r) {
            const int o = ch_of(r, h);
            if constexpr (VW0) {
                if (j == 0) {
                    red[o * CIN] = w0v[2 * r];
                    red[o * CIN + 1] = w0v[2 * r + 1];
                    red[32 * CIN + o] = b0v[r];
                }
            } else {
                if (j < CA) red[o * CIN + j] = dW0a[r];
                if (CB > 0 && j < CB) red[o * CIN + CA + j] = dW0b[r];
            }
        }
        int off = 32 * CIN;
#pragma unroll
        for (int l = 0; l < DEPTH; ++l) {
            if (l > 0) {
#pragma unroll
                for (int r = 0; r < 16; ++r) red[off + ch_of(r, h) * 32 + j] = dWh[l - 1][r];
                off += 1024;
            }
            if (h == 0 && !(VW0 && l == 0)) red[off + j] = db[l];
            off += 32;
        }
    }
    __syncthreads();
    static_assert(PCOUNT % 4 == 0, "partials are summed four at a time");
    float4 *out = reinterpret_cast<float4 *>(A.wpart + (long long)blockIdx.x * PCOUNT);
    const float4 *part4 = reinterpret_cast<const float4 *>(smem);
    for (int e = threadIdx.x; e < PCOUNT / 4; e += 64 * NW) {
        float4 a = part4[e];
#pragma unroll
        for (int w = 1; w < NW; ++w) {
            const float4 b = part4[w * (PCOUNT / 4) + e];
            a.x += b.x;
            a.y += b.y;
            a.z += b.z;
            a.w += b.w;
        }
        out[e] = a;
    }
}

template <int CA, int CB, bool PK, int NWT = 8>
int launch_bwd_x3(const fgnn_mlp_bwd_args *a, int tpg, int total, hipStream_t st) {
    constexpr int LDS = BwdX3Layout<CA, CB, NWT>::LDS_F * 4;
    constexpr int NW = NWT;
    static_assert(LDS <= 160 * 1024, "LDS budget");
    static LdsAttrCache attr_cache;
    (void)fgnn_raise_lds(attr_cache, (const void *)mlp_bwd_x3_kernel<CA, CB, PK, NWT>, LDS);
    hipLaunchKernelGGL((mlp_bwd_x3_kernel<CA, CB, PK, NWT>), dim3(a->cu_share == 2 ? BWD_WG / 2 : BWD_WG), dim3(64 * NW), LDS, st, *a, tpg, total);
    FGNN_LAUNCH_CHECK();
    return 0;
}

}

extern "C" int fgnn_mlp_bwd_x3(const fgnn_mlp_bwd_args *a, void *stream) {
    FGNN_CHECK(a != nullptr, "fgnn_mlp_bwd_x3: null args");
    FGNN_CHECK(a->G > 0 && a->N > 0, "fgnn_mlp_bwd_x3: bad G=%d N=%d", a->G, a->N);
    FGNN_CHECK(mlp_x3_supported(a->a.C, a->b.C, a->depth, 1),
               "fgnn_mlp_bwd_x3: built for depth 3 and 2, 32, 32+2, 32+32 input channels (got depth %d, %d + %d); use fgnn_mlp_bwd",
               a->depth, a->a.C, a->b.C);
    FGNN_CHECK(a->packed, "fgnn_mlp_bwd_x3: needs the operand image of fgnn_pack_x3_operands (kind 1)");
    FGNN_CHECK(!a->ranges, "fgnn_mlp_bwd_x3: no padding-tile skipping (ranges); use fgnn_mlp_bwd for ragged batches");
    FGNN_CHECK(BWD_WG == fgnn_mlp_bwd_num_workgroups(), "fgnn_mlp_bwd_x3: workgroup count differs from fgnn_mlp_bwd");
    const bool pk_a = a->xbits && a->a.C == 2, pk_b = a->xbits && a->b.C == 2;
    FGNN_CHECK((a->a.ptr || pk_a) && (a->b.C == 0 || a->b.ptr || pk_b), "fgnn_mlp_bwd_x3: slab pointer missing");
    FGNN_CHECK(!a->xbits || a->xdeg, "fgnn_mlp_bwd_x3: xbits without xdeg (fgnn_adjacency_degree)");
    FGNN_CHECK(!(a->a.C != 32 && a->dxa) && !(a->b.C != 32 && a->b.C != 0 && a->dxb),
               "fgnn_mlp_bwd_x3: input gradients exist for 32-channel slabs only; use fgnn_mlp_bwd");
    FGNN_CHECK(a->dy && a->z && a->wpart, "fgnn_mlp_bwd_x3: missing dy/z/wpart");
    FGNN_CHECK(a->coef || (a->s12 && a->znrm) || (a->s12tiles && a->znrm), "fgnn_mlp_bwd_x3: need coef, or s12 + znrm, or s12tiles + znrm");
    {
        const long long lim = 0x7fffffffll / 4, G = a->G;
        FGNN_CHECK(G * a->a.gstride < lim && G * a->b.gstride < lim && G * a->dgstride < lim && G * a->zgstride < lim &&
                   G * a->dxa_gstride < lim && G * a->dxb_gstride < lim,
                   "fgnn_mlp_bwd_x3: a tensor exceeds 2 GiB (32-bit buffer addressing); split the batch");
    }
    const int tpg = fgnn_tiles_per_graph(a->N);
    const long long total = (long long)a->G * tpg;
    FGNN_CHECK(total < (1ll << 30), "fgnn_mlp_bwd_x3: too many tiles");
    FGNN_CHECK(!a->s12tiles || a->b.C > 0, "fgnn_mlp_bwd_x3: s12tiles is built into the two-slab kernels only");
    FGNN_CHECK(!a->s12tiles || fgnn_mlp_bwd_coef_tiles_supported(a->G, a->N),
               "fgnn_mlp_bwd_x3: s12tiles needs a workgroup's tile range to span <= %d graphs (G=%d N=%d)", FGNN_BWD_COEF_GRAPHS, a->G, a->N);
    hipStream_t st = (hipStream_t)stream;
    const int ca = a->a.C, cb = a->b.C;
    if (a->xbits) {
        if (ca == 2 && cb == 0) return launch_bwd_x3<2, 0, true>(a, tpg, (int)total, st);
        if (ca == 32 && cb == 2) return launch_bwd_x3<32, 2, true>(a, tpg, (int)total, st);
        fgnn_set_error("fgnn_mlp_bwd_x3: xbits needs a 2-channel slab (2 or 32+2 input channels)");
        return 1;
    }
    if (ca == 2 && cb == 0) return launch_bwd_x3<2, 0, false>(a, tpg, (int)total, st);
    if (ca == 32 && cb == 0) return launch_bwd_x3<32, 0, false>(a, tpg, (int)total, st);
    if (ca == 32 && cb == 2) return launch_bwd_x3<32, 2, false>(a, tpg, (int)total, st);
    return launch_bwd_x3<32, 32, false>(a, tpg, (int)total, st);
}
```

### graph_neural_net_amd/csrc/pool_score.hip

```cpp
#include <float.h>
#include "fgnn_common.h"
#include "fgnn_norm.h"

namespace {

__global__ __launch_bounds__(256) void colmax_fwd_kernel(const fgnn_slab y, const int *nvalid, int G, int N, float *e,
                                                         int *idx) {
    const long long t = (long long)blockIdx.x * (blockDim.x / WAVE) + (threadIdx.x / WAVE);
    const int C = y.C;
    if (t >= (long long)G * C * N) return;
    const int lane = threadIdx.x & 63;
    const int i = (int)(t % N);
    const int gc = (int)(t / N);
    const int g = gc / C, c = gc - g * C;
    const int nv = nvalid_of(nvalid, g, N);
    float best = 0.f;
    int bi = 0;
    if (i < nv) {
        const float *row = y.ptr + (long long)g * y.gstride + (long long)c * y.ldp + (long long)i * N;
        float mean = 0.f, a = 1.f, be = 0.f;
        if (y.nrm) {
            const float4 n = reinterpret_cast<const float4 *>(y.nrm)[gc];
            mean = n.x;
            a = n.y;
// ... 175 lines not shown
    __shared__ int sidx[CMB_MAXN];
    __shared__ float sde[CMB_MAXN];
    __shared__ float red[4][2];
    const int gc = blockIdx.x, tid = threadIdx.x, lane = tid & 63, wave = tid >> 6;
    const int g = gc / C, c = gc - g * C;
    const int nv = nvalid_of(nvalid, g, N);
    float *mat = dy + (long long)g * gstride + (long long)c * ldp;
    const float *zm = s12 ? y.ptr + (long long)g * y.gstride + (long long)c * y.ldp : nullptr;
    const float mean = s12 ? y.nrm[(long long)gc * 4] : 0.f;
    const bool staged = N <= CMB_MAXN;
    float s1 = 0.f, s2 = 0.f;
    const bool late = N <= 256;
    float zlate = 0.f, dlate = 0.f;
    for (int i = tid; i < N; i += 256) {
        const long long t = (long long)gc * N + i;
        const int bi = idx[t];
        const float d = i < nv ? de[t] : 0.f;
        if (staged) {
            sidx[i] = bi;
            sde[i] = d;
        }
        if (s12 && i < nv) {
            if (late) {
                zlate = zm[(long long)i * N + bi];
                dlate = d;
            } else {
                s1 += d;
                s2 += d * (zm[(long long)i * N + bi] - mean);
            }
        }
    }
    __syncthreads();
    const float invN = 1.f / (float)N;
    if (staged && (ldp & 3) == 0 && (gstride & 3) == 0 && (reinterpret_cast<unsigned long long>(dy) & 15ull) == 0) {
        const int P = N * N;
        float4 *mat4 = reinterpret_cast<float4 *>(mat);
        for (int q = tid; 4 * q < P; q += 256) {
            const int p0 = 4 * q;
            int i = (int)(((float)p0 + 0.5f) * invN);
            int j = p0 - i * N;
            float v[4];
#pragma unroll
            for (int k = 0; k < 4; ++k) {
                const int ic = i < N ? i : 0;
                v[k] = (i < N && j == sidx[ic]) ? sde[ic] : 0.f;
                if (++j == N) {
                    j = 0;
                    ++i;
                }
            }
            if (p0 + 3 < P) {
                mat4[q] = make_float4(v[0], v[1], v[2], v[3]);
            } else {
#pragma unroll
                for (int k = 0; k < 4; ++k)
                    if (p0 + k < P) mat[p0 + k] = v[k];
            }
        }
    } else {
        for (int p = tid; p < N * N; p += 256) {
            const int i = (int)(((float)p + 0.5f) * invN);
            const int j = p - i * N;
            const int bi = staged ? sidx[i] : idx[(long long)gc * N + i];
            const float d = staged ? sde[i] : (i < nv ? de[(long long)gc * N + i] : 0.f);
            mat[p] = (j == bi) ? d : 0.f;
        }
    }
    if (s12) {
        if (late && tid < nv) {
            s1 += dlate;
            s2 += dlate * (zlate - mean);
        }
        s1 = wave_sum(s1);
        s2 = wave_sum(s2);
        if (lane == 0) {
            red[wave][0] = s1;
            red[wave][1] = s2;
        }
        __syncthreads();
        if (tid < 2) s12[(long long)gc * 2 + tid] = (red[0][tid] + red[1][tid]) + (red[2][tid] + red[3][tid]);
    }
}

DEVI void copy_to_lds256(float *dst, const float *src, int n, int tid) {
    constexpr int U = 8;
    int done = 0;
    if (((reinterpret_cast<unsigned long long>(src) | reinterpret_cast<unsigned long long>(dst)) & 15ull) == 0) {
        const int n4 = n >> 2;
        const float4 *s4 = reinterpret_cast<const float4 *>(src);
        float4 *d4 = reinterpret_cast<float4 *>(dst);
        for (int e0 = tid; e0 < n4; e0 += 256 * U) {
            float4 v[U];
#pragma unroll
            for (int k = 0; k < U; ++k) {
                const int e = e0 + 256 * k;
                v[k] = s4[e < n4 ? e : 0];
            }
#pragma unroll
            for (int k = 0; k < U; ++k) {
                const int e = e0 + 256 * k;
                if (e < n4) d4[e] = v[k];
            }
        }
        done = n4 << 2;
    }
    for (int e0 = done + tid; e0 < n; e0 += 256 * U) {
        float v[U];
#pragma unroll
        for (int k = 0; k < U; ++k) {
            const int e = e0 + 256 * k;
            v[k] = src[e < n ? e : 0];
        }
#pragma unroll
        for (int k = 0; k < U; ++k) {
            const int e = e0 + 256 * k;
            if (e < n) dst[e] = v[k];
        }
    }
}

__global__ __launch_bounds__(256) void score_ce_fwd_kernel(const float *e1, const float *e2, const int *nvalid,
                                                           int C, int N, int rows, float *scores, float *lse,
                                                           float *pair_loss) {
    extern __shared__ __attribute__((aligned(16))) float sm[];
    float *s2 = sm, *s1 = sm + (size_t)C * N;
    float *sS = s1 + (size_t)C * rows;
    float *red = sS + (size_t)rows * N;
    const int b = blockIdx.x, tid = threadIdx.x, lane = tid & 63, wave = tid >> 6;
    const int nv = nvalid_of(nvalid, b, N);
    const int i0 = blockIdx.y * rows;
    const int i1 = (i0 + rows < N) ? i0 + rows : N;
    const int w = i1 > i0 ? i1 - i0 : 0;
    const float *p1 = e1 + (long long)b * C * N, *p2 = e2 + (long long)b * C * N;
    copy_to_lds256(s2, p2, C * N, tid);
    for (int e = tid; e < C * w; e += 256) {
        const int c = e / w, r = e - c * w;
        s1[c * rows + r] = p1[c * N + i0 + r];
    }
    __syncthreads();
    float *S = scores + (long long)b * N * N;
    const float invN = 1.f / (float)N;
    for (int e = tid; e < w * N; e += 256) {
        const int r = (int)(((float)e + 0.5f) * invN), j = e - r * N;
        float acc = 0.f;
        if (i0 + r < nv && j < nv)
            for (int c = 0; c < C; ++c) acc = fmaf(s1[c * rows + r], s2[c * N + j], acc);
        S[(long long)i0 * N + e] = acc;
        sS[e] = acc;
    }
    __syncthreads();
    float wl = 0.f;
    for (int i = i0 + wave; i < i1; i += 4) {
        float l = 0.f;
        const float *Sr = sS + (size_t)(i - i0) * N;
        if (i < nv) {
            float mx = -FLT_MAX;
            for (int j = lane; j < nv; j += WAVE) mx = fmaxf(mx, Sr[j]);
            mx = wave_max(mx);
            float se = 0.f;
            for (int j = lane; j < nv; j += WAVE) se += expf(Sr[j] - mx);
            se = wave_sum(se);
            l = mx + logf(se);
            wl += l - Sr[i];
        }
        if (lane == 0 && lse) lse[(long long)b * N + i] = l;
    }
    if (lane == 0) red[wave] = wl;
    __syncthreads();
    if (tid == 0 && pair_loss) pair_loss[b * gridDim.y + blockIdx.y] = (red[0] + red[1]) + (red[2] + red[3]);
}

constexpr int CSPLIT = 4;
constexpr int CSPLIT_SMALL = 8;
template <bool CE, bool STAGE>
__global__ __launch_bounds__(256) void score_bwd_kernel(const float *e1, const float *e2, const float *scores,
                                                        const float *lse, const float *dscores, const int *nvalid,
                                                        const float *gscale, int C, int N, float *de1, float *de2) {
    extern __shared__ __attribute__((aligned(16))) float sm[];
    const int cper = (C + (int)gridDim.y - 1) / (int)gridDim.y;
    const int c0 = blockIdx.y * cper;
    const int cn = (c0 + cper <= C ? cper : (C > c0 ? C - c0 : 0));
    float *s1 = sm, *s2 = sm + (size_t)cper * N;
    float *dS = s2 + (size_t)cper * N;
    const int ld = N + 1;
    const int b = blockIdx.x, tid = threadIdx.x;
    const int nv = nvalid_of(nvalid, b, N);
    const float *p1 = e1 + ((long long)b * C + c0) * N, *p2 = e2 + ((long long)b * C + c0) * N;
    for (int e = tid; e < cn * N; e += 256) {
        s1[e] = p1[e];
        s2[e] = p2[e];
    }
    const float gs = CE ? *gscale : 1.f;
    const float *S = (CE ? scores : dscores) + (long long)b * N * N;
    const float *Lr = CE ? lse + (long long)b * N : nullptr;
    const float invN = 1.f / (float)N;
    auto ds_at = [&](int i, int jj) -> float {
        float d = S[(long long)i * N + jj];
        if (CE) d = (expf(d - Lr[i]) - (i == jj ? 1.f : 0.f)) * gs;
        return d;
    };
    if (STAGE) {
        constexpr int U = 8;
        for (int e0 = tid; e0 < N * N; e0 += 256 * U) {
            float v[U];
#pragma unroll
            for (int k = 0; k < U; ++k) {
                const int e = e0 + 256 * k;
                v[k] = S[e < N * N ? e : 0];
            }
#pragma unroll
            for (int k = 0; k < U; ++k) {
                const int e = e0 + 256 * k;
                if (e < N * N) {
                    const int i = (int)(((float)e + 0.5f) * invN);
                    const int jj = e - i * N;
                    float d = 0.f;
                    if (i < nv && jj < nv) {
                        d = v[k];
                        if (CE) d = (expf(d - Lr[i]) - (i == jj ? 1.f : 0.f)) * gs;
                    }
                    dS[i * ld + jj] = d;
                }
            }
        }
    }
    __syncthreads();
    for (int e = tid; e < cn * N; e += 256) {
        const int c = e / N, i = e - c * N;
        float a1 = 0.f, a2 = 0.f;
        if (i < nv) {
            const float *r2 = s2 + c * N, *r1 = s1 + c * N;
            for (int jj = 0; jj < nv; ++jj) {
                a1 = fmaf(r2[jj], STAGE ? dS[i * ld + jj] : ds_at(i, jj), a1);
                a2 = fmaf(r1[jj], STAGE ? dS[jj * ld + i] : ds_at(jj, i), a2);
            }
        }
        de1[((long long)b * C + c0) * N + e] = a1;
        de2[((long long)b * C + c0) * N + e] = a2;
    }
}

template <bool CE>
__global__ __launch_bounds__(256) void score_bwd_blocked_kernel(const float *e1, const float *e2, const float *scores,
                                                                const float *lse, const float *dscores,
                                                                const int *nvalid, const float *gscale, int C, int N,
                                                                int SB_BLK, float *de1, float *de2) {
    extern __shared__ __attribute__((aligned(16))) float sm[];
    const int cper = (C + CSPLIT - 1) / CSPLIT;
    const int c0 = blockIdx.y * cper;
    const int cn = (c0 + cper <= C ? cper : (C > c0 ? C - c0 : 0));
    float *s1 = sm, *s2 = sm + (size_t)cper * N;
    float *dS = s2 + (size_t)cper * N;
    const int b = blockIdx.x, tid = threadIdx.x;
    const int nv = nvalid_of(nvalid, b, N);
    const int x0 = blockIdx.z * SB_BLK, x1 = (x0 + SB_BLK < N) ? x0 + SB_BLK : N, w = x1 - x0;
    const float *p1 = e1 + ((long long)b * C + c0) * N, *p2 = e2 + ((long long)b * C + c0) * N;
    constexpr int U = 8;
    copy_to_lds256(s1, p1, cn * N, tid);
    copy_to_lds256(s2, p2, cn * N, tid);
    const float gs = CE ? *gscale : 1.f;
    const float *S = (CE ? scores : dscores) + (long long)b * N * N;
    const float *Lr = CE ? lse + (long long)b * N : nullptr;
    auto ds_of = [&](float sv, float lv, int i, int jj) -> float {
        if (i >= nv || jj >= nv) return 0.f;
        return CE ? (expf(sv - lv) - (i == jj ? 1.f : 0.f)) * gs : sv;
    };
    {
        const int ld = N + 1;
        for (int e0 = tid; e0 < w * N; e0 += 256 * U) {
            float sv[U], lv[U];
#pragma unroll
            for (int k = 0; k < U; ++k) {
                const int e = e0 + 256 * k, ec = e < w * N ? e : 0;
                const int r = ec / N;
                sv[k] = S[(long long)x0 * N + ec];
                lv[k] = CE ? Lr[x0 + r] : 0.f;
            }
#pragma unroll
            for (int k = 0; k < U; ++k) {
                const int e = e0 + 256 * k;
                if (e < w * N) {
                    const int r = e / N, jj = e - r * N;
                    dS[r * ld + jj] = ds_of(sv[k], lv[k], x0 + r, jj);
                }
            }
        }
        __syncthreads();
        for (int e = tid; e < cn * w; e += 256) {
            const int c = e / w, r = e - c * w;
            float a1 = 0.f;
            const float *r2 = s2 + c * N, *drow = dS + r * ld;
            for (int jj = 0; jj < nv; ++jj) a1 = fmaf(r2[jj], drow[jj], a1);
            de1[((long long)b * C + c0 + c) * N + x0 + r] = (x0 + r) < nv ? a1 : 0.f;
        }
        __syncthreads();
    }
    {
        const int ld = SB_BLK + 1;
        for (int e0 = tid; e0 < N * w; e0 += 256 * U) {
            float sv[U], lv[U];
#pragma unroll
            for (int k = 0; k < U; ++k) {
                const int e = e0 + 256 * k, ec = e < N * w ? e : 0;
                const int i = ec / w, r = ec - i * w;
                sv[k] = S[(long long)i * N + x0 + r];
                lv[k] = CE ? Lr[i] : 0.f;
            }
#pragma unroll
            for (int k = 0; k < U; ++k) {
// ... 27 lines not shown
        if (i < nv) {
            float mx = -FLT_MAX;
            for (int j = lane; j < nv; j += WAVE) mx = fmaxf(mx, S[(long long)i * N + j]);
            mx = wave_max(mx);
            float se = 0.f;
            for (int j = lane; j < nv; j += WAVE) se += expf(S[(long long)i * N + j] - mx);
            se = wave_sum(se);
            l = mx + logf(se);
            wl += l - S[(long long)i * N + i];
        }
        if (lane == 0 && lse) lse[(long long)b * N + i] = l;
    }
    if (lane == 0) red[wave] = wl;
    __syncthreads();
    if (tid == 0 && pair_loss) pair_loss[b] = (red[0] + red[1]) + (red[2] + red[3]);
}

__global__ void ce_bwd_kernel(const float *scores, const float *lse, const int *nvalid, const float *gscale, int N,
                              float *dscores) {
    const int b = blockIdx.y;
    const int e = blockIdx.x * blockDim.x + threadIdx.x;
    if (e >= N * N) return;
    const int nv = nvalid_of(nvalid, b, N);
    const int i = e / N, j = e - i * N;
    float d = 0.f;
    if (i < nv && j < nv)
        d = (expf(scores[(long long)b * N * N + e] - lse[(long long)b * N + i]) - (i == j ? 1.f : 0.f)) * (*gscale);
    dscores[(long long)b * N * N + e] = d;
}

}

extern "C" int fgnn_colmax_fwd(const fgnn_slab *y, const int *nvalid, int G, int N, float *e, int *idx, void *stream) {
    FGNN_CHECK(y && y->ptr && e && idx && G > 0 && N > 0 && y->C > 0, "fgnn_colmax_fwd: bad arguments");
    const long long tot = (long long)G * y->C * N;
    if (N <= 64) {
        hipLaunchKernelGGL(colmax_fwd_lds_kernel<false>, dim3((unsigned)((G * y->C + 3) / 4)), dim3(256), 0,
                           (hipStream_t)stream, *y, nvalid, G, N, e, idx, ColmaxFin{});
        FGNN_LAUNCH_CHECK();
        return 0;
    }
    if (N <= 128) {
        hipLaunchKernelGGL(colmax_fwd_rows16_kernel<8>, dim3((unsigned)((tot + 15) / 16)), dim3(256), 0, (hipStream_t)stream, *y, nvalid, G, N, e, idx);
        FGNN_LAUNCH_CHECK();
        return 0;
    }
    if (N <= 256) {
        hipLaunchKernelGGL(colmax_fwd_rows16_kernel<16>, dim3((unsigned)((tot + 15) / 16)), dim3(256), 0, (hipStream_t)stream, *y, nvalid, G, N, e, idx);
        FGNN_LAUNCH_CHECK();
        return 0;
    }
    hipLaunchKernelGGL(colmax_fwd_kernel, dim3((unsigned)((tot + 3) / 4)), dim3(256), 0, (hipStream_t)stream, *y,
                       nvalid, G, N, e, idx);
    FGNN_LAUNCH_CHECK();
    return 0;
}

extern "C" int fgnn_colmax_fwd_fin_supported(int N) { return N <= 64 ? 1 : 0; }

extern "C" int fgnn_colmax_fwd_fin(const fgnn_slab *y, const float *part, const float *cnt, const float *gn_weight, float eps,
                                   const int *nvalid, int G, int N, float *e, int *idx, void *stream) {
    FGNN_CHECK(y && y->ptr && y->nrm && part && cnt && e && idx && G > 0 && N > 0 && y->C > 0, "fgnn_colmax_fwd_fin: bad arguments");
    FGNN_CHECK(N <= 64, "fgnn_colmax_fwd_fin: N=%d > 64 (use fgnn_gn_finalize + fgnn_colmax_fwd)", N);
    const ColmaxFin F = {part, cnt, gn_weight, eps, fgnn_tiles_per_graph(N)};
    hipLaunchKernelGGL(colmax_fwd_lds_kernel<true>, dim3((unsigned)((G * y->C + 3) / 4)), dim3(256), 0, (hipStream_t)stream, *y,
                       nvalid, G, N, e, idx, F);
    FGNN_LAUNCH_CHECK();
    return 0;
}

extern "C" int fgnn_colmax_bwd(const float *de, const int *idx, const int *nvalid, int G, int C, int N, float *dy,
                               long long gstride, long long ldp, const fgnn_slab *y, float *s12, void *stream) {
    FGNN_CHECK(de && idx && dy && G > 0 && C > 0 && N > 0, "fgnn_colmax_bwd: bad arguments");
    FGNN_CHECK(!s12 || (y && y->ptr && y->nrm && y->C == C), "fgnn_colmax_bwd: s12 needs the normalised input slab");
    fgnn_slab ys = {};
    if (s12) ys = *y;
    const int tot = G * C;
    hipLaunchKernelGGL(colmax_bwd_kernel, dim3((unsigned)tot), dim3(256), 0, (hipStream_t)stream, de,
                       idx, nvalid, G, C, N, dy, gstride, ldp, ys, s12);
    FGNN_LAUNCH_CHECK();
    return 0;
}

static int score_lds_bytes(int C, int N) { return (2 * C * N + 4) * (int)sizeof(float); }
static int score_bwd_lds_bytes(int C, int N, bool stage, int csplit = CSPLIT) {
    const int cper = (C + csplit - 1) / csplit;
    return (2 * cper * N + (stage ? N * (N + 1) : 0)) * (int)sizeof(float);
}
template <bool CE>
static int launch_score_bwd(const float *e1, const float *e2, const float *scores, const float *lse,
                            const float *dscores, const int *nvalid, const float *gscale, int B, int C, int N,
                            float *de1, float *de2, hipStream_t st) {
    const bool stage = score_bwd_lds_bytes(C, N, true) <= 160 * 1024 && (N <= 64 || (long long)B * CSPLIT >= 256);
    const int csplit = (long long)B * CSPLIT < 256 ? CSPLIT_SMALL : CSPLIT;
    const int lds = score_bwd_lds_bytes(C, N, stage, stage ? csplit : CSPLIT);
    FGNN_CHECK(lds <= 160 * 1024, "score backward: C*N=%d too large for LDS staging", C * N);
    if (stage) {
        if (lds > 64 * 1024)
            (void)hipFuncSetAttribute((const void *)score_bwd_kernel<CE, true>, hipFuncAttributeMaxDynamicSharedMemorySize, lds);
        hipLaunchKernelGGL((score_bwd_kernel<CE, true>), dim3(B, csplit), dim3(256), lds, st, e1, e2, scores, lse, dscores,
                           nvalid, gscale, C, N, de1, de2);
    } else {
        const int cper = (C + CSPLIT - 1) / CSPLIT;
        const int SB_BLK = (long long)B * CSPLIT * ((N + 63) / 64) >= 512 ? 64 : 16;
        const int big = (N + 1) * SB_BLK > N * (SB_BLK + 1) ? (N + 1) * SB_BLK : N * (SB_BLK + 1);
        const int lds2 = (2 * cper * N + big) * (int)sizeof(float);
        FGNN_CHECK(lds2 <= 160 * 1024, "score backward: N=%d too large for the blocked LDS staging", N);
        if (lds2 > 64 * 1024)
            (void)hipFuncSetAttribute((const void *)score_bwd_blocked_kernel<CE>, hipFuncAttributeMaxDynamicSharedMemorySize, lds2);
        hipLaunchKernelGGL((score_bwd_blocked_kernel<CE>), dim3(B, CSPLIT, (N + SB_BLK - 1) / SB_BLK), dim3(256), lds2, st, e1, e2,
                           scores, lse, dscores, nvalid, gscale, C, N, SB_BLK, de1, de2);
    }
    FGNN_LAUNCH_CHECK();
    return 0;
}

extern "C" int fgnn_score_row_blocks(int B, int N) {
    if (B * FGNN_SCORE_SPLIT >= 512) return FGNN_SCORE_SPLIT;
    return (N + 3) / 4;
}

extern "C" int fgnn_score_ce_fwd_blocks(const float *e1, const float *e2, const int *nvalid, int B, int C, int N,
                                        int row_blocks, float *scores, float *lse, float *pair_loss, void *stream) {
    FGNN_CHECK(e1 && e2 && scores && B > 0 && C > 0 && N > 0 && row_blocks > 0, "fgnn_score_ce_fwd: bad arguments");
    const int rows = (N + row_blocks - 1) / row_blocks;
    const int lds = (C * N + C * rows + rows * N + 4) * (int)sizeof(float);
    FGNN_CHECK(lds <= 160 * 1024, "fgnn_score_ce_fwd: C*N=%d too large for LDS staging", C * N);
    if (lds > 64 * 1024)
        (void)hipFuncSetAttribute((const void *)score_ce_fwd_kernel, hipFuncAttributeMaxDynamicSharedMemorySize, lds);
    hipLaunchKernelGGL(score_ce_fwd_kernel, dim3(B, row_blocks), dim3(256), lds, (hipStream_t)stream, e1, e2, nvalid, C, N, rows,
                       scores, lse, pair_loss);
    FGNN_LAUNCH_CHECK();
    return 0;
}

extern "C" int fgnn_score_ce_fwd(const float *e1, const float *e2, const int *nvalid, int B, int C, int N,
                                 float *scores, float *lse, float *pair_loss, void *stream) {
    return fgnn_score_ce_fwd_blocks(e1, e2, nvalid, B, C, N, FGNN_SCORE_SPLIT, scores, lse, pair_loss, stream);
}

extern "C" int fgnn_score_ce_bwd(const float *e1, const float *e2, const float *scores, const float *lse,
                                 const int *nvalid, const float *gscale, int B, int C, int N, float *de1, float *de2,
                                 void *stream) {
    FGNN_CHECK(e1 && e2 && scores && lse && gscale && de1 && de2 && B > 0, "fgnn_score_ce_bwd: bad arguments");
    return launch_score_bwd<true>(e1, e2, scores, lse, nullptr, nvalid, gscale, B, C, N, de1, de2, (hipStream_t)stream);
}

extern "C" int fgnn_score_bwd(const float *e1, const float *e2, const float *dscores, const int *nvalid, int B, int C,
                              int N, float *de1, float *de2, void *stream) {
    FGNN_CHECK(e1 && e2 && dscores && de1 && de2 && B > 0, "fgnn_score_bwd: bad arguments");
    return launch_score_bwd<false>(e1, e2, nullptr, nullptr, dscores, nvalid, nullptr, B, C, N, de1, de2, (hipStream_t)stream);
}

extern "C" int fgnn_ce_fwd(const float *scores, const int *nvalid, int B, int N, float *lse, float *pair_loss,
                           void *stream) {
    FGNN_CHECK(scores && lse && pair_loss && B > 0 && N > 0, "fgnn_ce_fwd: bad arguments");
    hipLaunchKernelGGL(ce_fwd_kernel, dim3(B), dim3(256), 0, (hipStream_t)stream, scores, nvalid, N, lse, pair_loss);
    FGNN_LAUNCH_CHECK();
    return 0;
}

extern "C" int fgnn_ce_bwd(const float *scores, const float *lse, const int *nvalid, const float *gscale, int B, int N,
                           float *dscores, void *stream) {
    FGNN_CHECK(scores && lse && gscale && dscores && B > 0 && N > 0, "fgnn_ce_bwd: bad arguments");
    hipLaunchKernelGGL(ce_bwd_kernel, dim3((N * N + 255) / 256, B), dim3(256), 0, (hipStream_t)stream, scores, lse,
                       nvalid, gscale, N, dscores);
    FGNN_LAUNCH_CHECK();
    return 0;
}
```

### graph_neural_net_amd/engine.py

```python
import ctypes as C
import os

import torch

from . import _lib

EPS = 1e-05


class ParamLayout:

    def __init__(self, original_features_num=2, num_blocks=4, in_features=32, out_features=32, depth_of_mlp=3):
        if in_features != _lib.FGNN_H or out_features != _lib.FGNN_H:
            raise RuntimeError('the fused engine is built for in_features = out_features = 32 (got %d, %d); other widths '
                               'run through the per-layer modules (layers.MlpBlock_Real)' % (in_features, out_features))
        if not 1 <= depth_of_mlp <= _lib.FGNN_MAX_DEPTH:
            raise RuntimeError('depth_of_mlp must be in 1..%d' % _lib.FGNN_MAX_DEPTH)
        if original_features_num not in (2, 32):
            raise RuntimeError('the fused engine is built for original_features_num = 2 or 32 (got %d); other widths run '
                               'through the per-layer modules (layers.MlpBlock_Real)' % original_features_num)
        self.c0 = original_features_num
        self.num_blocks = num_blocks
        self.depth = depth_of_mlp
        self.entries = []
# ... 53 lines not shown
def _numel(shape):
    n = 1
    for s in shape:
        n *= s
    return n


def _round_up(x, m):
    return (x + m - 1) // m * m


class EngineCache:

    def __init__(self, budget):
        import collections
        self.budget = budget
        self._items = collections.OrderedDict()

    @staticmethod
    def engine_bytes(G, N, num_blocks, elt=4):
        ldp = -(-N * N // 32) * 32
        return (4 * num_blocks + 5) * G * 32 * ldp * elt

    def get(self, key, factory, nbytes):
        hit = self._items.get(key)
        if hit is not None:
            self._items.move_to_end(key)
            return hit[0], []
        eng = factory()
        self._items[key] = (eng, nbytes)
        evicted = []
        while self.used() > self.budget and len(self._items) > 1:
            k, _ = self._items.popitem(last=False)
            evicted.append(k)
        return eng, evicted

    def used(self):
        return sum(b for _, b in self._items.values())

    def keys(self):
        return list(self._items)

    def clear(self):
        self._items.clear()

    def __len__(self):
        return len(self._items)

    def __iter__(self):
        return iter(list(self._items))

    def values(self):
        return [e for e, _ in self._items.values()]


class FgnnEngine:
    SKIP_PADDING_TILES = True
    MM_ORDER = True
    PAIR_BWD = os.environ.get('FGNN_PAIR_BWD', '1') != '0'
    PACK_IN_STRUCT = os.environ.get('FGNN_PACK_IN_STRUCT', '1') != '0'
    T16 = os.environ.get('FGNN_T16', 'pair,bwd')

    MFMA = os.environ.get('FGNN_MFMA', 'f32')

    BLOCK1 = os.environ.get('FGNN_BLOCK1', 'generic')

    def __init__(self, layout, G, N, device, ragged=False, cu_share=0, mfma=None, block1=None):
        _lib.load()
        self.T16 = type(self).T16
        self.cu_share = int(cu_share)
        mfma = self.MFMA if mfma is None else mfma
        if mfma not in ('f32', 'x3'):
            raise ValueError("mfma must be 'f32' or 'x3' (got %r)" % (mfma,))
        self.x3 = (mfma == 'x3' and not ragged and layout.depth == 3 and layout.c0 in (2, 32))
        block1 = self.BLOCK1 if block1 is None else block1
        if block1 not in ('generic', 'structured'):
            raise ValueError("block1 must be 'generic' or 'structured' (got %r)" % (block1,))
        self.struct1 = (block1 == 'structured' and cu_share == 0
                        and bool(_lib.load().fgnn_block1_struct_supported(N, layout.depth, layout.c0)))
        self._struct = None
        self.decisions = None
        self.layout = layout
        self.G, self.N = G, N
        self.P = N * N
        self.ldp = _round_up(self.P, 32)
        self.tpg = _lib.tiles_per_graph(N)
        self.device = device
        K = layout.num_blocks
        f32 = dict(dtype=torch.float32, device=device)
        act = lambda: torch.empty(G * 32 * self.ldp, **f32)
        self.z = {(k, j): act() for k in range(1, K + 1) for j in (1, 2, 3)}
        self.mult = {k: act() for k in range(1, K + 1)}
        self.nrm = {(k, j): torch.empty(G * 32 * 4, **f32) for k in range(1, K + 1) for j in (1, 2, 3)}
        self.part = [torch.empty(G * self.tpg * 32 * 2, **f32) for _ in range(2)]
        self.cnt = torch.empty(G * 2 * self.tpg, **f32)
        self.E = torch.empty(G, 32, N, **f32)
        self.idx = torch.empty(G, 32, N, dtype=torch.int32, device=device)
        self.B = G // 2
        self.scores = torch.empty(self.B, N, N, **f32)
        self.lse = torch.empty(self.B, N, **f32)
        self.score_blocks = _lib.load().fgnn_score_row_blocks(self.B, N)
        self.pair_loss = torch.empty(self.B * self.score_blocks, **f32)
        self.loss = torch.empty(1, **f32)
        self.nvalid = torch.empty(G, dtype=torch.int32, device=device) if ragged else None
        self._nvalid_own = self.nvalid
        self.ranges = (torch.empty(_lib.FGNN_RANGE_WG + 1, dtype=torch.int32, device=device)
                       if ragged and self.SKIP_PADDING_TILES else None)
        self.mm_order = (torch.empty(G, dtype=torch.int32, device=device)
                         if self.ranges is not None and self.MM_ORDER and 64 < N <= 256 else None)
        self._bwd = None
        self.x = None
        self.xbits = None
        self.xdeg = None
        self._packs = {}
        for k in range(1, K + 1):
            cin = layout.c0 if k == 1 else 32
            fl = _lib.load().fgnn_pack_x3_floats if self.x3 else _lib.load().fgnn_pack_floats
            f12, b12 = 0, (5 if self._t16_pair(cin) else 1)
            f3 = 2 if self.x3 else 0
            b3 = 5 if self._t16_bwd3(cin) else (3 if self.x3 else 1)
            self._packs[('f', k, 12)] = (f12, cin, 0, 2, torch.empty(fl(f12, cin, 0, layout.depth, 2), **f32))
            self._packs[('f', k, 3)] = (f3, 32, cin, 1, torch.empty(fl(f3, 32, cin, layout.depth, 1), **f32))
            for j in (1, 2):
                self._packs[('b', k, j)] = (b12, cin, 0, 1, torch.empty(fl(b12, cin, 0, layout.depth, 1), **f32))
            self._packs[('b', k, 3)] = (b3, 32, cin, 1, torch.empty(fl(b3, 32, cin, layout.depth, 1), **f32))

    def _t16(self, what):
        return self.T16 not in ('0', '') and what in self.T16.split(',')

    def _t16_pair(self, cin):
        return (self._t16('pair') and self.PAIR_BWD and not self.x3 and self.layout.depth == 3 and cin == 32 and self.N <= 256)

    def _t16_bwd3(self, cin):
        return self._t16('bwd') and not self.x3 and self.layout.depth == 3 and cin in (2, 32) and self.N <= 256

    def _nv(self):
        return _lib.ptr(self.nvalid) if self.nvalid is not None else None

    def _w(self, params, off):
        return params.data_ptr() + 4 * off

    def _slab_in(self, k, params):
        if k == 1:
            if self.xbits is not None:
                s = _lib.Slab()
                s.gstride, s.ldp, s.C = self.layout.c0 * self.P, self.P, self.layout.c0
                return s
            return _lib.make_slab(self.x, self.layout.c0 * self.P, self.P, self.layout.c0)
        rec = self.layout.mlp[(k - 1, 3)]
        s = _lib.make_slab(self.z[(k - 1, 3)], 32 * self.ldp, self.ldp, 32, nrm=self.nrm[(k - 1, 3)])
        s.beta = self._w(params, rec['gn_b'])
        return s

    def _slab_z(self, k, j, params):
        rec = self.layout.mlp[(k, j)]
        s = _lib.make_slab(self.z[(k, j)], 32 * self.ldp, self.ldp, 32, nrm=self.nrm[(k, j)])
        s.beta = self._w(params, rec['gn_b'])
        return s

    def _slab_raw(self, t):
        return _lib.make_slab(t, 32 * self.ldp, self.ldp, 32)

    def pack_operands(self, params):
        L = self.layout
        self._pack_launch(params, list(self._packs.items()), 'fgnn_pack_x3_operands' if self.x3 else 'fgnn_pack_operands')

# ... 125 lines not shown
            self._mlp_fwd(params, k, (3,), self._slab_raw(self.mult[k]), sin, finalize=not pool_fin)
        out = self._slab_z(L.num_blocks, 3, params)
        if pool_fin:
            rec = L.mlp[(L.num_blocks, 3)]
            _lib.call('fgnn_colmax_fwd_fin', C.byref(out), _lib.ptr(self.part[0]), _lib.ptr(self.cnt),
                      C.c_void_p(self._w(params, rec['gn_w'])), EPS, self._nv(), self.G, self.N, _lib.ptr(self.E),
                      _lib.ptr(self.idx), st, tag='fgnn_colmax_fwd')
        else:
            _lib.call('fgnn_colmax_fwd', C.byref(out), self._nv(), self.G, self.N, _lib.ptr(self.E), _lib.ptr(self.idx), st)
        return self.E

    def _fill(self):
        return 1 if self.ranges is not None else 0

    def _struct_ws(self):
        if self._struct is None:
            lib = _lib.load()
            f32 = dict(dtype=torch.float32, device=self.device)
            self._struct = {'tab': torch.empty(lib.fgnn_block1_struct_table_floats(self.N), **f32),
                            'ws': torch.empty(lib.fgnn_block1_struct_ws_floats(self.G, self.N), **f32)}
        return self._struct

    def _w3(self, params, j):
        rec = self.layout.mlp[(1, j)]
        return ((C.c_void_p * 3)(*[self._w(params, o) for o in rec['w']]), (C.c_void_p * 3)(*[self._w(params, o) for o in rec['b']]))

    def _struct_fwd(self, params, with_pack=False):
        S = self._struct_ws()
        st = _lib.stream_ptr()
        (w1, b1), (w2, b2) = self._w3(params, 1), self._w3(params, 2)
        r1, r2 = self.layout.mlp[(1, 1)], self.layout.mlp[(1, 2)]
        args = [_lib.ptr(self.xbits), self._nv(), self.G, self.N, _lib.ptr(S['tab']),
                C.c_void_p(self._w(params, r1['gn_w'])), C.c_void_p(self._w(params, r1['gn_b'])),
                C.c_void_p(self._w(params, r2['gn_w'])), C.c_void_p(self._w(params, r2['gn_b'])), EPS,
                _lib.ptr(self.nrm[(1, 1)]), _lib.ptr(self.nrm[(1, 2)]), _lib.ptr(self.mult[1]), 32 * self.ldp, self.ldp,
                _lib.ptr(self.xdeg), _lib.ptr(S['ws']), w1, b1, w2, b2]
        if with_pack:
            items = list(self._packs.items())
            _lib.call('fgnn_block1_struct_fwd_pack', *args, self._pack_jobs(params, items), len(items), st)
        else:
            _lib.call('fgnn_block1_struct_fwd', *args, st)

    def _struct_bwd(self, params):
        S, W = self._struct_ws(), self._bwd
        W['struct_rows'] = int(_lib.load().fgnn_block1_struct_rows(self.G, self.N))
        (w1, _), (w2, _) = self._w3(params, 1), self._w3(params, 2)
        r1, r2 = self.layout.mlp[(1, 1)], self.layout.mlp[(1, 2)]
        _lib.call('fgnn_block1_struct_bwd', _lib.ptr(self.xbits), self._nv(), self.G, self.N, _lib.ptr(S['tab']), w1, w2,
                  _lib.ptr(self.nrm[(1, 1)]), _lib.ptr(self.nrm[(1, 2)]),
                  C.c_void_p(self._w(params, r1['gn_b'])), C.c_void_p(self._w(params, r2['gn_b'])),
                  _lib.ptr(W['dmult']), 32 * self.ldp, self.ldp, _lib.ptr(S['ws']),
                  _lib.ptr(W['wpart'][(1, 1)]), _lib.ptr(W['wpart'][(1, 2)]), _lib.ptr(W['s12'][(1, 1)]), _lib.ptr(W['s12'][(1, 2)]),
                  _lib.stream_ptr())

    def forward(self, params, x, nvalid=None, total_nodes=None, defer_loss=False, loss_out=None, bits=None, pack=True):
        self.embed(params, x, nvalid, bits=bits, pack=pack)
        B, N = self.B, self.N
        st = _lib.stream_ptr()
        e1, e2 = self.E[:B], self.E[B:]
        if total_nodes is None:
            total_nodes = B * N if nvalid is None else int(nvalid[:B].sum().item())
        self.total_nodes = float(total_nodes)
        _lib.call('fgnn_score_ce_fwd_blocks', _lib.ptr(e1), _lib.ptr(e2), self._nv(), B, 32, N, self.score_blocks,
                  _lib.ptr(self.scores), _lib.ptr(self.lse), _lib.ptr(self.pair_loss), st)
        self._loss_pending = bool(defer_loss)
        self._loss_target = self.loss if loss_out is None else loss_out
        if not defer_loss:
            _lib.call('fgnn_sum_scale', _lib.ptr(self.pair_loss), B * self.score_blocks, 1, 1.0 / self.total_nodes,
                      _lib.ptr(self._loss_target), st)
        return self.scores, self._loss_target

    def _alloc_bwd(self):
        if self._bwd is not None:
            return self._bwd
        f32 = dict(dtype=torch.float32, device=self.device)
        act = lambda: torch.empty(self.G * 32 * self.ldp, **f32)
        nwg = _lib.load().fgnn_mlp_bwd_num_workgroups()
        if self.cu_share == 2 and self.ranges is None:
            nwg //= 2
        L = self.layout
        keys = [(k, j) for k in range(1, L.num_blocks + 1) for j in (1, 2, 3)]
        self._bwd = {
            'dE': torch.empty(self.G, 32, self.N, **f32),
            'dy': [act(), act()],
            'dmult': act(), 'dy1': act(), 'dy2': act(),
            's12': {kj: torch.empty(self.G * 32 * 2, **f32) for kj in keys},
            'wpart': {kj: torch.empty(nwg * L.mlp[kj]['count'], **f32)
                      for kj in keys},
            's12part': torch.empty(self.G * self.tpg * 32 * 2, **f32),
            'coef': [torch.empty(self.G * 32 * 4, **f32) for _ in range(3)],
            'nwg': nwg,
            'gscale': torch.empty(1, **f32),
        }
        return self._bwd

    def _coef(self, kj, slot):
        W = self._bwd
        _lib.call('fgnn_gn_bwd_coef', _lib.ptr(W['s12'][kj]), _lib.ptr(self.nrm[kj]), self._nv(), self.G, 32, self.N,
                  _lib.ptr(W['coef'][slot]), None, None, _lib.stream_ptr())

    def _mlp_bwd(self, params, k, j, a, b, dy, coef, dxa, dxb, acc_a, acc_b, emit=False, dx_strides=None):
        args = self._mlp_bwd_args(params, k, j, a, b, dy, coef, dxa, dxb, acc_a, acc_b, emit, dx_strides)
        entry = 'fgnn_mlp_bwd_x3' if (self.x3 and j != 3) else 'fgnn_mlp_bwd'
        if j == 3 and b is not None and self._t16_bwd3(b.C) and _lib.load().fgnn_mlp_bwd_t16_supported(C.byref(args)):
            entry = 'fgnn_mlp_bwd_t16'
        elif self._packs[('b', k, j)][0] == 5:
            args.packed = None
        _lib.call(entry, C.byref(args), _lib.stream_ptr(),
                  tag='mlp_bwd[cin=%d,dx=%d]' % (a.C + (b.C if b is not None else 0),
                                                (a.C if dxa is not None else 0) + (b.C if (b is not None and dxb is not None) else 0)))

    def _mlp_bwd_pair(self, params, k, sin, din, emit):
        W = self._bwd
        a1 = self._mlp_bwd_args(params, k, 1, sin, None, W['dy1'], None, None, None, False, False, False, None)
        a2 = self._mlp_bwd_args(params, k, 2, sin, None, W['dy2'], None, din, None, True, False, emit, None)
        entry = 'fgnn_mlp_bwd_pair_x3' if self.x3 else ('fgnn_mlp_bwd_pair_t16' if self._t16_pair(sin.C) else 'fgnn_mlp_bwd_pair')
        _lib.call(entry, C.byref(a1), C.byref(a2), _lib.stream_ptr(),
                  tag='mlp_bwd_pair[cin=%d,dx=%d]' % (sin.C, sin.C if din is not None else 0))

    def _mlp_bwd_args(self, params, k, j, a, b, dy, coef, dxa, dxb, acc_a, acc_b, emit, dx_strides):
        L = self.layout
        W = self._bwd
        rec = L.mlp[(k, j)]
        gs = 32 * self.ldp
        args = _lib.MlpBwdArgs()
        args.G, args.N, args.depth = self.G, self.N, L.depth
        args.nvalid = self.nvalid.data_ptr() if self.nvalid is not None else None
        args.a = a
        if b is not None:
            args.b = b
        for l in range(L.depth):
            args.W[l] = self._w(params, rec['w'][l])
            args.bias[l] = self._w(params, rec['b'][l])
        args.dy, args.dgstride, args.ldd = dy.data_ptr(), gs, self.ldp
        args.z, args.zgstride, args.ldz = self.z[(k, j)].data_ptr(), gs, self.ldp
        if isinstance(coef, str):
            args.s12tiles = W['s12part'].data_ptr()
            args.s12_out = W['s12'][(k, j)].data_ptr()
            args.znrm = self.nrm[(k, j)].data_ptr()
        elif coef is not None:
            args.coef = coef.data_ptr()
        else:
            args.s12 = W['s12'][(k, j)].data_ptr()
            args.znrm = self.nrm[(k, j)].data_ptr()
        dgs, dld = (gs, self.ldp) if dx_strides is None else dx_strides
        if dxa is not None:
            args.dxa, args.dxa_gstride, args.dxa_ld = dxa.data_ptr(), (gs if (b is not None and dx_strides is not None) else dgs), \
                (self.ldp if (b is not None and dx_strides is not None) else dld)
        if dxb is not None:
            args.dxb, args.dxb_gstride, args.dxb_ld = dxb.data_ptr(), dgs, dld
        args.accumulate_a, args.accumulate_b = int(acc_a), int(acc_b)
        args.wpart = W['wpart'][(k, j)].data_ptr()
        args.packed = self._packs[('b', k, j)][4].data_ptr()
        self._packed_input(args, k)
        if self.ranges is not None:
            args.ranges = self.ranges.data_ptr()
        args.cu_share = self.cu_share
        if emit:
            args.s12part = W['s12part'].data_ptr()
        return args

    def backward(self, params, grads, grad_scale=1.0, finalize=True, gscale_dev=None):
        W = self._alloc_bwd()
        B, N = self.B, self.N
        st = _lib.stream_ptr()
        gs_t = W['gscale']
        if gscale_dev is not None:
            gs_t = gscale_dev
        else:
            self._set_gscale(grad_scale / self.total_nodes)
        e1, e2 = self.E[:B], self.E[B:]
        _lib.call('fgnn_score_ce_bwd', _lib.ptr(e1), _lib.ptr(e2), _lib.ptr(self.scores), _lib.ptr(self.lse),
                  self._nv(), _lib.ptr(gs_t), B, 32, N, _lib.ptr(W['dE'][:B]), _lib.ptr(W['dE'][B:]), st)
        return self.backward_from_dE(params, grads, W['dE'], finalize=finalize)

    def _set_gscale(self, gs):
        W = self._bwd
        if W.get('gscale_value') != gs:
            W['gscale'].fill_(gs)
            W['gscale_value'] = gs

    def backward_from_dE(self, params, grads, dE, finalize=True, dx=None):
        L = self.layout
        W = self._alloc_bwd()
        st = _lib.stream_ptr()
        gs = 32 * self.ldp
        K = L.num_blocks
        in_prologue = bool(_lib.load().fgnn_mlp_bwd_coef_tiles_supported(self.G, self.N)) and self.ranges is None
        dy = W['dy'][0]
        out = self._slab_z(K, 3, params)
        _lib.call('fgnn_colmax_bwd', _lib.ptr(dE), _lib.ptr(self.idx), self._nv(), self.G, 32, self.N,
                  _lib.ptr(dy), gs, self.ldp, C.byref(out), _lib.ptr(W['s12'][(K, 3)]), st)
        for k in range(K, 0, -1):
            sin = self._slab_in(k, params)
            first = (k == 1)
            din = None if first else W['dy'][(K - k + 1) % 2]
            dxs = None
            if first and dx is not None:
                if self.xbits is not None or self.x3 or tuple(dx.shape) != (self.G, L.c0, self.N, self.N) or dx.dtype != torch.float32 \
                        or not dx.is_contiguous():
                    raise RuntimeError('FgnnEngine: the input gradient needs a dense fp32 input, the fp32-MFMA kernels (mfma="f32") '
                                       'and a contiguous (G, c0, N, N) fp32 dx')
                din, dxs = dx, (L.c0 * self.P, self.P)
            self._mlp_bwd(params, k, 3, self._slab_raw(self.mult[k]), sin, dy,
                          None if k == K else ('tiles' if in_prologue else W['coef'][2]), W['dmult'], din, False, False, dx_strides=dxs)
            if first and self.struct1 and self.xbits is not None and dxs is None:
                self._struct_bwd(params)
                dy = din
                continue
            ya, yb = self._slab_z(k, 1, params), self._slab_z(k, 2, params)
            _lib.call('fgnn_chan_matmul_bwd_ord', C.byref(ya), C.byref(yb), _lib.ptr(W['dmult']), gs, self.ldp,
                      self._nv(), self.G, self.N, _lib.ptr(W['dy1']), _lib.ptr(W['dy2']), gs, self.ldp,
                      _lib.ptr(W['s12'][(k, 1)]), _lib.ptr(W['s12'][(k, 2)]),
                      _lib.ptr(self.mm_order) if self.mm_order is not None else None, self._fill(), st, tag='fgnn_chan_matmul_bwd')
            if first:
                W['struct_rows'] = 0
            if self.PAIR_BWD and dxs is None and L.depth == 3 and sin.C in (2, 32):
                self._mlp_bwd_pair(params, k, sin, din, emit=not first)
            else:
                self._mlp_bwd(params, k, 1, sin, None, W['dy1'], None, din, None, True, False, dx_strides=dxs)
                self._mlp_bwd(params, k, 2, sin, None, W['dy2'], None, din, None, True, False, emit=not first, dx_strides=dxs)
            if not first and not in_prologue:
                _lib.call('fgnn_gn_bwd_coef_tiles', _lib.ptr(W['s12part']), _lib.ptr(self.nrm[(k - 1, 3)]), self._nv(),
                          self.G, 32, self.N, _lib.ptr(W['s12'][(k - 1, 3)]), _lib.ptr(W['coef'][2]), st)
            dy = din
        if finalize:
            self.grad_finalize(grads)
        return grads

    def grad_finalize(self, grads, rows=None, graphs=None, pair_rows=None):
        L = self.layout
        W = self._bwd
        K = L.num_blocks
        st = _lib.stream_ptr()
        keys = [(k, j) for k in range(1, K + 1) for j in (1, 2, 3)]
        if getattr(self, '_loss_pending', False):
            keys.append('loss')
            self._loss_pending = False
        for lo in range(0, len(keys), _lib.MAX_GRAD_JOBS):
            chunk = keys[lo:lo + _lib.MAX_GRAD_JOBS]
            jobs = (_lib.GradJob * len(chunk))()
            for i, kj in enumerate(chunk):
                if kj == 'loss':
                    jobs[i].wpart = self.pair_loss.data_ptr()
                    jobs[i].count = 1
                    jobs[i].out = self._loss_target.data_ptr()
                    jobs[i].rows = self.B * self.score_blocks if pair_rows is None else pair_rows
                    jobs[i].scale = 1.0 / self.total_nodes
                    if getattr(self, '_loss_scale_dev', None) is not None:
                        jobs[i].scale_dev = self._loss_scale_dev.data_ptr()
                    continue
                rec = L.mlp[kj]
                jobs[i].wpart = W['wpart'][kj].data_ptr()
                jobs[i].count = rec['count']
                if kj in ((1, 1), (1, 2)) and W.get('struct_rows', 0):
                    jobs[i].rows = W['struct_rows']
                jobs[i].out = grads.data_ptr() + 4 * rec['off']
                jobs[i].s12 = W['s12'][kj].data_ptr()
                jobs[i].nrm = self.nrm[kj].data_ptr()
                jobs[i].dgn_w = grads.data_ptr() + 4 * rec['gn_w']
                jobs[i].dgn_b = grads.data_ptr() + 4 * rec['gn_b']
            _lib.call('fgnn_grad_finalize', jobs, len(chunk), W['nwg'] if rows is None else rows,
                      self.G if graphs is None else graphs, 32, st)
        return grads

    def step(self, params, grads, x, nvalid=None, total_nodes=None, loss_out=None, bits=None):
        scores, loss = self.forward(params, x, nvalid, total_nodes, defer_loss=True, loss_out=loss_out, bits=bits)
        self.backward(params, grads)
        return scores, loss

    def export_decisions(self, on=True):
        self.decisions = {} if on else None

    def relu_decisions(self, params=None):
        L, G, N, P = self.layout, self.G, self.N, self.P
        out = {}
        bit = torch.arange(32, device=self.device, dtype=torch.int32)
        for (k, j), buf in self.decisions.items():
            w = buf.view(G, L.depth - 1, 32, self.tpg)
            m = ((w.unsqueeze(-1) >> bit) & 1).reshape(G, L.depth - 1, 32, self.tpg * 32)[..., :P].reshape(G, L.depth - 1, 32, N, N)
            for l in range(L.depth - 1):
                out[(k, j, l)] = m[:, l].bool()
        if self.struct1 and self.xbits is not None and (1, 1) not in self.decisions:
            nc = 2 + 2 * (N + 1)
            tab = self._struct['tab'].view(2, nc, 4, 32)
            words = (N + 31) // 32
            b = self.xbits.view(G, N, words).to(torch.int64) & 0xffffffff
            col = torch.arange(N, device=self.device)
# ... 27 lines not shown
```

### include/fgnn_hip.h

```cpp
#ifndef FGNN_HIP_H
#define FGNN_HIP_H

#ifdef __cplusplus
extern "C" {
#endif

#define FGNN_H 32
#define FGNN_TILE 32
#define FGNN_MAX_DEPTH 3

typedef struct {
    const float *ptr;
    long long gstride;
    long long ldp;
    int C;
    const float *nrm;
    const float *beta;
} fgnn_slab;

const char *fgnn_last_error(void);
int fgnn_version(void);
int fgnn_tiles_per_graph(int N);
int fgnn_mlp_bwd_num_workgroups(void);

// ... 72 lines not shown
    int M, K;
    int relu;
    const float *mask;
    float *out;
    long long o_gstride;
} fgnn_chain_layer;
typedef struct {
    const float *x;
    long long x_gstride, x_ld;
    int depth;
    fgnn_chain_layer layer[3];
    long long o_ld;
    const int *nvalid;
    int G, N;
} fgnn_chain_args;
int fgnn_conv_chain_supported(int depth, int K0, const int *M );
int fgnn_conv_chain(const fgnn_chain_args *args, void *stream);

typedef struct {
    const float *x;
    long long x_gstride, x_ld;
    int cin;
    const float *xb;
    long long xb_gstride, xb_ld;
    int cb;
    const float *packed;
    const int *nvalid;
    int G, N;
    float *out;
    long long o_gstride, o_ld;
    const float *dz;
    long long dz_gstride, dz_ld;
    float *dx;
    long long dx_gstride, dx_ld;
    float *dxb;
    long long dxb_gstride, dxb_ld;
    int accumulate_dx, accumulate_dxb;
    float *wpart;
} fgnn_mlp64_args;
int fgnn_mlp64_supported(int cin, int depth, int width);
int fgnn_mlp64_num_workgroups(void);
int fgnn_mlp64_param_count(int cin);
int fgnn_mlp64_packed_floats(int cin);
int fgnn_mlp64_pack(const float *W0, const float *W1, const float *W2, const float *b0, const float *b1, const float *b2, int cin,
                    float *packed, void *stream);
typedef struct {
    const float *W[3];
    const float *bias[3];
    int cin;
    float *packed;
} fgnn_mlp64_pack_job;
int fgnn_mlp64_pack_multi(const fgnn_mlp64_pack_job *jobs, int njobs, void *stream);
int fgnn_mlp64_fwd(const fgnn_mlp64_args *args, void *stream);
int fgnn_mlp64_bwd(const fgnn_mlp64_args *args, void *stream);

int fgnn_chan_matmul_fwd(const fgnn_slab *ya, const fgnn_slab *yb, const int *nvalid, int G, int N,
                         float *out, long long ogstride, long long ldo, void *stream);
int fgnn_chan_matmul_fwd_ord(const fgnn_slab *ya, const fgnn_slab *yb, const int *nvalid, int G, int N,
                             float *out, long long ogstride, long long ldo, const int *order, int fill, void *stream);
int fgnn_chan_matmul_fwd_fin_supported(int N);
int fgnn_chan_matmul_fwd_fin(const fgnn_slab *ya, const fgnn_slab *yb, const float *part_a, const float *part_b,
                             const float *cnt, const float *gn_weight_a, const float *gn_weight_b, float eps,
                             const int *nvalid, int G, int N, float *out, long long ogstride, long long ldo, void *stream);
int fgnn_chan_matmul_fwd_fin_ord(const fgnn_slab *ya, const fgnn_slab *yb, const float *part_a, const float *part_b,
                                 const float *cnt, const float *gn_weight_a, const float *gn_weight_b, float eps,
                                 const int *nvalid, int G, int N, float *out, long long ogstride, long long ldo,
                                 const int *order , int fill, void *stream);

int fgnn_colmax_fwd(const fgnn_slab *y, const int *nvalid, int G, int N, float *e ,
                    int *idx , void *stream);
int fgnn_colmax_fwd_fin_supported(int N);
int fgnn_colmax_fwd_fin(const fgnn_slab *y, const float *part, const float *cnt, const float *gn_weight, float eps,
                        const int *nvalid, int G, int N, float *e, int *idx, void *stream);

#define FGNN_SCORE_SPLIT 4
int fgnn_score_ce_fwd(const float *e1, const float *e2, const int *nvalid, int B, int C, int N,
                      float *scores, float *lse, float *pair_loss, void *stream);
int fgnn_score_row_blocks(int B, int N);
int fgnn_score_ce_fwd_blocks(const float *e1, const float *e2, const int *nvalid, int B, int C, int N, int row_blocks,
                             float *scores, float *lse, float *pair_loss, void *stream);
int fgnn_score_ce_bwd(const float *e1, const float *e2, const float *scores, const float *lse,
                      const int *nvalid, const float *gscale, int B, int C, int N,
                      float *de1, float *de2, void *stream);

int fgnn_ce_fwd(const float *scores, const int *nvalid, int B, int N, float *lse, float *pair_loss, void *stream);
int fgnn_ce_bwd(const float *scores, const float *lse, const int *nvalid, const float *gscale, int B, int N,
                float *dscores, void *stream);
int fgnn_score_bwd(const float *e1, const float *e2, const float *dscores, const int *nvalid,
                   int B, int C, int N, float *de1, float *de2, void *stream);

int fgnn_colmax_bwd(const float *de, const int *idx, const int *nvalid, int G, int C, int N,
                    float *dy, long long gstride, long long ldp, const fgnn_slab *y, float *s12, void *stream);

int fgnn_gn_bwd_stats(const float *dy, long long dgstride, long long ldd,
                      const float *z, long long zgstride, long long ldz, const float *nrm,
                      const int *nvalid, int G, int C, int N, float *s12 , void *stream);
int fgnn_gn_bwd_coef(const float *s12, const float *nrm, const int *nvalid, int G, int C, int N,
                     float *coef , float *dgn_w , float *dgn_b ,
                     void *stream);
int fgnn_gn_bwd_coef_tiles(const float *s12part, const float *nrm, const int *nvalid, int G, int C, int N,
                           float *s12, float *coef, void *stream);
int fgnn_gn_bwd_apply(const float *dy, long long dgstride, long long ldd,
                      const float *z, long long zgstride, long long ldz, const float *coef,
                      const int *nvalid, int G, int C, int N, float *dz, long long ogstride, long long ldo, void *stream);

typedef struct {
    int G, N, depth;
    const int *nvalid;
    fgnn_slab a, b;
    const float *W[FGNN_MAX_DEPTH];
    const float *bias[FGNN_MAX_DEPTH];
    const float *dy;  long long dgstride, ldd;
    const float *z;   long long zgstride, ldz;
    const float *coef;
    const float *s12;
    const float *znrm;
    float *dxa; long long dxa_gstride, dxa_ld;
    float *dxb; long long dxb_gstride, dxb_ld;
    int accumulate_a, accumulate_b;
    float *wpart;
    float *s12part;
    const float *packed;
    const float *s12tiles;
    float *s12_out;
    const unsigned *xbits;
    const float *xdeg;
    const int *ranges;
    int cu_share;
} fgnn_mlp_bwd_args;
int fgnn_mlp_bwd(const fgnn_mlp_bwd_args *args, void *stream);
int fgnn_mlp_bwd_x3(const fgnn_mlp_bwd_args *args, void *stream);
int fgnn_mlp_bwd_pair(const fgnn_mlp_bwd_args *m1, const fgnn_mlp_bwd_args *m2, void *stream);
int fgnn_mlp_bwd_pair_x3(const fgnn_mlp_bwd_args *m1, const fgnn_mlp_bwd_args *m2, void *stream);
int fgnn_mlp_bwd_t16_supported(const fgnn_mlp_bwd_args *args);
int fgnn_mlp_bwd_t16(const fgnn_mlp_bwd_args *args, void *stream);
int fgnn_mlp_bwd_pair_t16(const fgnn_mlp_bwd_args *m1, const fgnn_mlp_bwd_args *m2, void *stream);
#define FGNN_BWD_COEF_GRAPHS 4
int fgnn_mlp_bwd_coef_tiles_supported(int G, int N);
int fgnn_mlp_param_count(int Cin, int depth);
int fgnn_reduce_partials(const float *wpart, int num_wg, int count, float *out, void *stream);

#define FGNN_MAX_GRAD_JOBS 16
typedef struct {
    const float *wpart; int count; float *out;
    const float *s12; const float *nrm; float *dgn_w; float *dgn_b;
    int rows;
    float scale;
    const float *scale_dev;
} fgnn_grad_job;
int fgnn_grad_finalize(const fgnn_grad_job *jobs, int njobs, int num_wg, int G, int C, void *stream);
int fgnn_inv_node_count(const int *nvalid, int B, float *out, void *stream);

int fgnn_chan_matmul_bwd(const fgnn_slab *ya, const fgnn_slab *yb, const float *dm, long long dmgstride, long long ldm,
                         const int *nvalid, int G, int N,
                         float *da, float *db, long long ogstride, long long ldo,
                         float *s12a ,
                         float *s12b , void *stream);
int fgnn_chan_matmul_bwd_ord(const fgnn_slab *ya, const fgnn_slab *yb, const float *dm, long long dmgstride, long long ldm,
                             const int *nvalid, int G, int N, float *da, float *db, long long ogstride, long long ldo,
                             float *s12a, float *s12b, const int *order, int fill , void *stream);

int fgnn_adam_step(float *params, const float *grads, float *exp_avg, float *exp_avg_sq, int n, double lr,
                   double beta1, double beta2, double eps, int step, double grad_scale, void *stream);
int fgnn_adam_step_dev(float *params, const float *grads, float *exp_avg, float *exp_avg_sq, int n,
                       const double *hp, int *state, void *stream);
int fgnn_accuracy_max(const float *scores, const int *nvalid, int B, int N, int *correct, void *stream);
#define FGNN_LSAP_MAX_N 2048
int fgnn_lsap_accuracy(const float *cost, long long bstride, int ld, const int *nvalid, int B, int N, int *correct,
                       int *assign , void *stream);

int fgnn_block1_struct_supported(int N, int depth, int original_features_num);
int fgnn_block1_struct_table_floats(int N);
long long fgnn_block1_struct_ws_floats(int G, int N);
int fgnn_block1_struct_rows(int G, int N);
int fgnn_block1_struct_fwd(const unsigned *bits, const int *nvalid, int G, int N, const float *tables, const float *gnw1, const float *gnb1,
                           const float *gnw2, const float *gnb2, float eps, float *nrm1, float *nrm2, float *mult, long long gstride,
                           long long ldp, float *xdeg , float *ws,
                           const float *const *tW1, const float *const *tb1, const float *const *tW2, const float *const *tb2
                           ,
                           void *stream);
int fgnn_block1_struct_bwd(const unsigned *bits, const int *nvalid, int G, int N, const float *tables, const float *const *W1,
                           const float *const *W2, const float *nrm1, const float *nrm2, const float *gnb1, const float *gnb2,
                           const float *dmult, long long gstride, long long ldp, float *ws, float *wpart1, float *wpart2, float *s12_1,
                           float *s12_2, void *stream);
int fgnn_block1_struct_fwd_pack(const unsigned *bits, const int *nvalid, int G, int N, const float *tables, const float *gnw1, const float *gnb1,
                                const float *gnw2, const float *gnb2, float eps, float *nrm1, float *nrm2, float *mult, long long gstride,
                                long long ldp, float *xdeg, float *ws, const float *const *tW1, const float *const *tb1,
                                const float *const *tW2, const float *const *tb2, const fgnn_pack_job *jobs, int njobs, void *stream);
int fgnn_block1_struct_fwd16(const unsigned *bits, const int *nvalid, int G, int N, int ldr, const float *tables, const float *gnw1,
                             const float *gnb1, const float *gnw2, const float *gnb2, float eps, float *nrm1, float *nrm2,
                             void *mult , long long gstride, long long ldp, void *x16 , float *ws,
                             const float *const *tW1, const float *const *tb1, const float *const *tW2, const float *const *tb2, void *stream);
int fgnn_block1_struct_fwd16_pack(const unsigned *bits, const int *nvalid, int G, int N, int ldr, const float *tables, const float *gnw1,
                                  const float *gnb1, const float *gnw2, const float *gnb2, float eps, float *nrm1, float *nrm2, void *mult,
                                  long long gstride, long long ldp, void *x16, float *ws, const float *const *tW1, const float *const *tb1,
                                  const float *const *tW2, const float *const *tb2, const fgnn_pack_job *jobs, int njobs, void *stream);
int fgnn_block1_struct_bwd16(const unsigned *bits, const int *nvalid, int G, int N, int ldr, const float *tables, const float *const *W1,
                             const float *const *W2, const float *nrm1, const float *nrm2, const float *gnb1, const float *gnb2,
                             const void *dmult , long long gstride, long long ldp, float *ws, float *wpart1, float *wpart2,
                             float *s12_1, float *s12_2, void *stream);

int fgnn_expand_adjacency(const unsigned *bits, const int *nvalid, int G, int N, float *x, void *stream);
int fgnn_pack_adjacency(const float *x, const int *nvalid, int G, int N, unsigned *bits, int *bad, void *stream);
int fgnn_pack_adjacency_ld(const float *x, const int *nvalid, int G, int Nin, int N, unsigned *bits, int *bad, void *stream);
int fgnn_pack_adjacency_pair(const float *x1, const float *x2, const int *nvalid1, const int *nvalid2, int B, int Nin, int N, unsigned *bits,
                             int *nv_out, float *inv_out, int *bad, void *stream);
int fgnn_adjacency_degree(const unsigned *bits, const int *nvalid, int G, int N, float *deg, void *stream);

#define FGNN_RANGE_WG 256
int fgnn_ragged_tile_ranges(const int *nvalid, int G, int N, int *ranges , void *stream);
int fgnn_ragged_tile_ranges_order(const int *nvalid, int G, int N, int *ranges , int *order ,
                                  void *stream);
// ... 116 lines not shown
```

Before: 42350.

## Fuse score/CE backward with colmax backward into compact dy records

Adds a record form of the pooled gradient: for each (graph, channel, column) it stores the gradient value together with its argmax row index as a float2. This replaces the dense N×N dy scatter that colmax backward produced. The score/CE backward kernel now also emits these records and the group-norm s12 sums, so separate dE and colmax_bwd passes are no longer needed. The t16 MLP backward kernel reads the records and rebuilds the sparse dy in registers by masking on the column index. This trades a larger, mostly-zero dy tensor and an extra launch for a few extra loads and compares per element; it only applies for N<=64 with the t16 path.

Result: faster. 42780 (median of 6 runs) (+1.0%).

```diff
diff --git a/graph_neural_net_amd/_lib.py b/graph_neural_net_amd/_lib.py
--- a/graph_neural_net_amd/_lib.py
+++ b/graph_neural_net_amd/_lib.py
@@ -80,7 +80,7 @@
                 ('accumulate_a', C.c_int), ('accumulate_b', C.c_int),
                 ('wpart', C.c_void_p), ('s12part', C.c_void_p), ('packed', C.c_void_p),
                 ('s12tiles', C.c_void_p), ('s12_out', C.c_void_p), ('xbits', C.c_void_p), ('xdeg', C.c_void_p),
-                ('ranges', C.c_void_p), ('cu_share', C.c_int)]
+                ('ranges', C.c_void_p), ('cu_share', C.c_int), ('dy_records', C.c_int)]
 
 
 class Slab16(C.Structure):
@@ -182,11 +182,13 @@
     'fgnn_score_row_blocks': [_I, _I],
     'fgnn_score_ce_fwd_blocks': [_VP, _VP, _VP, _I, _I, _I, _I, _VP, _VP, _VP, _VP],
     'fgnn_score_ce_bwd': [_VP, _VP, _VP, _VP, _VP, _VP, _I, _I, _I, _VP, _VP, _VP],
+    'fgnn_score_ce_bwd_rec': [_VP, _VP, _VP, _VP, _VP, _VP, _I, _I, _I, _VP, C.POINTER(Slab), _VP, _VP, _VP],
     'fgnn_inv_node_count': [_VP, _I, _VP, _VP],
     'fgnn_score_bwd': [_VP, _VP, _VP, _VP, _I, _I, _I, _VP, _VP, _VP],
     'fgnn_ce_fwd': [_VP, _VP, _I, _I, _VP, _VP, _VP],
     'fgnn_ce_bwd': [_VP, _VP, _VP, _VP, _I, _I, _VP, _VP],
     'fgnn_colmax_bwd': [_VP, _VP, _VP, _I, _I, _I, _VP, _LL, _LL, C.POINTER(Slab), _VP, _VP],
+    'fgnn_colmax_bwd_rec': [_VP, _VP, _VP, _I, _I, _I, _VP, C.POINTER(Slab), _VP, _VP],
     'fgnn_gn_bwd_stats': [_VP, _LL, _LL, _VP, _LL, _LL, _VP, _VP, _I, _I, _I, _VP, _VP],
     'fgnn_gn_bwd_coef': [_VP, _VP, _VP, _I, _I, _I, _VP, _VP, _VP, _VP],
     'fgnn_gn_bwd_coef_tiles': [_VP, _VP, _VP, _I, _I, _I, _VP, _VP, _VP],
diff --git a/graph_neural_net_amd/csrc/mlp_bwd.hip b/graph_neural_net_amd/csrc/mlp_bwd.hip
--- a/graph_neural_net_amd/csrc/mlp_bwd.hip
+++ b/graph_neural_net_amd/csrc/mlp_bwd.hip
@@ -734,6 +734,7 @@
 
 extern "C" int fgnn_mlp_bwd(const fgnn_mlp_bwd_args *a, void *stream) {
     FGNN_CHECK(a != nullptr, "fgnn_mlp_bwd: null args");
+    FGNN_CHECK(!a->dy_records, "fgnn_mlp_bwd: dy_records is a form of fgnn_mlp_bwd_t16");
     FGNN_CHECK(a->G > 0 && a->N > 0, "fgnn_mlp_bwd: bad G=%d N=%d", a->G, a->N);
     FGNN_CHECK(a->depth >= 1 && a->depth <= FGNN_MAX_DEPTH, "fgnn_mlp_bwd: depth %d not in 1..%d", a->depth, FGNN_MAX_DEPTH);
     const bool pk_a = a->xbits && a->a.C == 2, pk_b = a->xbits && a->b.C == 2;
diff --git a/graph_neural_net_amd/csrc/mlp_bwd_pair.hip b/graph_neural_net_amd/csrc/mlp_bwd_pair.hip
--- a/graph_neural_net_amd/csrc/mlp_bwd_pair.hip
+++ b/graph_neural_net_amd/csrc/mlp_bwd_pair.hip
@@ -466,6 +466,7 @@
 
 extern "C" int fgnn_mlp_bwd_pair(const fgnn_mlp_bwd_args *a1, const fgnn_mlp_bwd_args *a2, void *stream) {
     FGNN_CHECK(a1 && a2, "fgnn_mlp_bwd_pair: null args");
+    FGNN_CHECK(!a1->dy_records && !a2->dy_records, "fgnn_mlp_bwd_pair: dy_records is a form of fgnn_mlp_bwd_t16");
     FGNN_CHECK(BWD_WG == fgnn_mlp_bwd_num_workgroups(), "fgnn_mlp_bwd_pair: workgroup count differs from fgnn_mlp_bwd");
     FGNN_CHECK(a1->G > 0 && a1->N > 0 && a1->G == a2->G && a1->N == a2->N && a1->depth == a2->depth,
                "fgnn_mlp_bwd_pair: the two MLPs must share G, N and depth");
diff --git a/graph_neural_net_amd/csrc/mlp_bwd_pair_t16.hip b/graph_neural_net_amd/csrc/mlp_bwd_pair_t16.hip
--- a/graph_neural_net_amd/csrc/mlp_bwd_pair_t16.hip
+++ b/graph_neural_net_amd/csrc/mlp_bwd_pair_t16.hip
@@ -442,6 +442,7 @@
 
 extern "C" int fgnn_mlp_bwd_pair_t16(const fgnn_mlp_bwd_args *a1, const fgnn_mlp_bwd_args *a2, void *stream) {
     FGNN_CHECK(a1 && a2, "fgnn_mlp_bwd_pair_t16: null args");
+    FGNN_CHECK(!a1->dy_records && !a2->dy_records, "fgnn_mlp_bwd_pair_t16: dy_records is a form of fgnn_mlp_bwd_t16");
     FGNN_CHECK(BWD_WG == fgnn_mlp_bwd_num_workgroups() && BWD_WG == FGNN_RANGE_WG, "fgnn_mlp_bwd_pair_t16: workgroup count differs from fgnn_mlp_bwd");
     FGNN_CHECK(a1->G > 0 && a1->N > 0 && a1->G == a2->G && a1->N == a2->N && a1->depth == a2->depth,
                "fgnn_mlp_bwd_pair_t16: the two MLPs must share G, N and depth");
diff --git a/graph_neural_net_amd/csrc/mlp_bwd_pair_x3.hip b/graph_neural_net_amd/csrc/mlp_bwd_pair_x3.hip
--- a/graph_neural_net_amd/csrc/mlp_bwd_pair_x3.hip
+++ b/graph_neural_net_amd/csrc/mlp_bwd_pair_x3.hip
@@ -465,6 +465,7 @@
 
 extern "C" int fgnn_mlp_bwd_pair_x3(const fgnn_mlp_bwd_args *a1, const fgnn_mlp_bwd_args *a2, void *stream) {
     FGNN_CHECK(a1 && a2, "fgnn_mlp_bwd_pair_x3: null args");
+    FGNN_CHECK(!a1->dy_records && !a2->dy_records, "fgnn_mlp_bwd_pair_x3: dy_records is a form of fgnn_mlp_bwd_t16");
     FGNN_CHECK(BWD_WG == fgnn_mlp_bwd_num_workgroups(), "fgnn_mlp_bwd_pair_x3: workgroup count differs from fgnn_mlp_bwd");
     FGNN_CHECK(a1->G > 0 && a1->N > 0 && a1->G == a2->G && a1->N == a2->N && a1->depth == a2->depth,
                "fgnn_mlp_bwd_pair_x3: the two MLPs must share G, N and depth");
diff --git a/graph_neural_net_amd/csrc/mlp_bwd_t16.hip b/graph_neural_net_amd/csrc/mlp_bwd_t16.hip
--- a/graph_neural_net_amd/csrc/mlp_bwd_t16.hip
+++ b/graph_neural_net_amd/csrc/mlp_bwd_t16.hip
@@ -42,7 +42,7 @@
     static constexpr int LDS_F = MAIN_F > RED_F ? MAIN_F : RED_F;
 };
 
-template <int CB, bool PKD, bool SKIP, bool DXB>
+template <int CB, bool PKD, bool SKIP, bool DXB, bool VDY>
 __global__ __launch_bounds__(64 * NW, 2) void mlp_bwd_t16_kernel(const fgnn_mlp_bwd_args A, const int tpg, const int total_tiles) {
     extern __shared__ __attribute__((aligned(16))) float smem[];
     using L = Layout16<CB>;
@@ -54,7 +54,7 @@
     const View vb = make_view(A.b.ptr, A.b.gstride, A.b.ldp, A.G);
     PackedSrc ps = {};
     if constexpr (PKD) ps = make_packed_src(A.xbits, A.xdeg, A.G, A.N);
-    const View vdy = make_view(A.dy, A.dgstride, A.ldd, A.G);
+    const View vdy = VDY ? make_view(A.dy, 64ll * A.N, 2ll * A.N, A.G) : make_view(A.dy, A.dgstride, A.ldd, A.G);
     const View vz = make_view(A.z, A.zgstride, A.ldz, A.G);
     const View vdxa = make_view(A.dxa, A.dxa_gstride, A.dxa_ld, A.G);
     const View vdxb = make_view(A.dxb, A.dxb_gstride, A.dxb_ld, A.G);
@@ -176,6 +176,7 @@
 
     constexpr int NXB = CB == 32 ? 8 : 1;
     float xa[8], xb[NXB], dyr[8], zr[8];
+    int dyi[VDY ? 8 : 1];
     auto load_x = [&](int h) {
         const bool act = h < H1;
         const int g = __builtin_amdgcn_readfirstlane(act ? h / hpg : 0);
@@ -201,7 +202,19 @@
         const int g = __builtin_amdgcn_readfirstlane(act ? h / hpg : 0);
         const int p = (act ? h - g * hpg : 0) * 16 + px;
         const bool inb = act && p < P2;
-        load8(dyr, vdy, lane_voff(vdy, q, p, inb), g * vdy.gs4);
+        if constexpr (VDY) {
+            int i, jj;
+            row_col(p, A.N, rcpN, i, jj);
+            const int voff = inb ? chan_q(q) * vdy.ld4 + 8 * i : OOB_OFF;
+#pragma unroll
+            for (int s = 0; s < 8; ++s) {
+                const auto r = __builtin_amdgcn_raw_buffer_load_b64(vdy.r, voff, g * vdy.gs4 + chan_s(s) * vdy.ld4, 0);
+                dyr[s] = __builtin_bit_cast(float, r[0]);
+                dyi[s] = (int)r[1];
+            }
+        } else {
+            load8(dyr, vdy, lane_voff(vdy, q, p, inb), g * vdy.gs4);
+        }
         load8(zr, vz, lane_voff(vz, q, p, inb), g * vz.gs4);
     };
 
@@ -311,6 +324,12 @@
             stage8(S1, lane_base, h2);
         }
         float dpre[8];
+        if constexpr (VDY) {
+            int i, jj;
+            row_col(p, A.N, rcpN, i, jj);
+#pragma unroll
+            for (int s = 0; s < 8; ++s) dyr[s] = dyi[s] == jj ? dyr[s] : 0.f;
+        }
 #pragma unroll
         for (int s = 0; s < 8; ++s) dpre[s] = fmaf(kz[s], zr[s] - kx[s], fmaf(ky[s], dyr[s], kw[s]));
         if (!full) {
@@ -433,13 +452,13 @@
     }
 }
 
-template <int CB, bool PKD, bool SKIP, bool DXB>
+template <int CB, bool PKD, bool SKIP, bool DXB, bool VDY = false>
 int launch16(const fgnn_mlp_bwd_args *a, int tpg, int total, hipStream_t st) {
     constexpr int LDS = Layout16<CB>::LDS_F * 4;
     static_assert(LDS <= 160 * 1024, "LDS budget");
     static LdsAttrCache attr_cache;
-    (void)fgnn_raise_lds(attr_cache, (const void *)mlp_bwd_t16_kernel<CB, PKD, SKIP, DXB>, LDS);
-    hipLaunchKernelGGL((mlp_bwd_t16_kernel<CB, PKD, SKIP, DXB>), dim3(a->cu_share == 2 && !SKIP ? BWD_WG / 2 : BWD_WG), dim3(64 * NW), LDS, st, *a,
+    (void)fgnn_raise_lds(attr_cache, (const void *)mlp_bwd_t16_kernel<CB, PKD, SKIP, DXB, VDY>, LDS);
+    hipLaunchKernelGGL((mlp_bwd_t16_kernel<CB, PKD, SKIP, DXB, VDY>), dim3(a->cu_share == 2 && !SKIP ? BWD_WG / 2 : BWD_WG), dim3(64 * NW), LDS, st, *a,
                        tpg, total);
     FGNN_LAUNCH_CHECK();
     return 0;
@@ -454,14 +473,15 @@
 extern "C" int fgnn_mlp_bwd_t16_supported(const fgnn_mlp_bwd_args *a) {
     if (!a || a->depth != 3 || a->a.C != 32 || a->a.nrm || !a->dxa || a->accumulate_a || a->accumulate_b || !a->packed || a->N > 256) return 0;
     if (a->b.C == 32) return (a->b.nrm && a->dxb && !a->xbits) ? 1 : 0;
-    if (a->b.C == 2) return (!a->b.nrm && !a->dxb) ? 1 : 0;
+    if (a->b.C == 2) return (!a->b.nrm && !a->dxb && !a->dy_records) ? 1 : 0;
     return 0;
 }
 
 extern "C" int fgnn_mlp_bwd_t16(const fgnn_mlp_bwd_args *a, void *stream) {
     FGNN_CHECK(a != nullptr, "fgnn_mlp_bwd_t16: null args");
     FGNN_CHECK(fgnn_mlp_bwd_t16_supported(a), "fgnn_mlp_bwd_t16: built for depth 3, slab a = 32 raw channels with dx stored, slab b = 32 normalised "
-               "channels with dx stored or 2 raw channels without dx, an operand image of kind 5, N <= 256; use fgnn_mlp_bwd");
+               "channels with dx stored or 2 raw channels without dx (and without dy_records), an operand image of kind 5, N <= 256; use fgnn_mlp_bwd");
+    const bool rec = a->dy_records != 0;
     FGNN_CHECK(a->G > 0 && a->N > 0 && a->a.ptr && (a->b.ptr || (a->xbits && a->b.C == 2)), "fgnn_mlp_bwd_t16: bad G / N / slabs");
     FGNN_CHECK(!a->xbits || a->xdeg, "fgnn_mlp_bwd_t16: xbits without xdeg (fgnn_adjacency_degree)");
     FGNN_CHECK(a->dy && a->z && a->wpart, "fgnn_mlp_bwd_t16: missing dy/z/wpart");
@@ -469,8 +489,8 @@
     FGNN_CHECK(BWD_WG == fgnn_mlp_bwd_num_workgroups() && BWD_WG == FGNN_RANGE_WG, "fgnn_mlp_bwd_t16: workgroup count differs from fgnn_mlp_bwd");
     {
         const long long lim = 0x7fffffffll / 4, G = a->G;
-        FGNN_CHECK(G * a->a.gstride < lim && G * a->b.gstride < lim && G * a->dgstride < lim && G * a->zgstride < lim &&
-                   G * a->dxa_gstride < lim && G * a->dxb_gstride < lim,
+        FGNN_CHECK(G * a->a.gstride < lim && G * a->b.gstride < lim && (rec || G * a->dgstride < lim) && G * a->zgstride < lim &&
+                   G * a->dxa_gstride < lim && G * a->dxb_gstride < lim && (!rec || G * 64 * a->N < lim),
                    "fgnn_mlp_bwd_t16: a tensor exceeds 2 GiB (32-bit buffer addressing); split the batch");
     }
     for (int l = 0; l < a->depth; ++l) FGNN_CHECK(a->W[l] && a->bias[l], "fgnn_mlp_bwd_t16: missing weights layer %d", l);
@@ -481,6 +501,7 @@
     FGNN_CHECK(!a->s12tiles || fgnn_mlp_bwd_coef_tiles_supported(a->G, a->N), "fgnn_mlp_bwd_t16: s12tiles needs a workgroup's tile range to span <= %d graphs",
                FGNN_BWD_COEF_GRAPHS);
     hipStream_t st = (hipStream_t)stream;
+    if (rec) return a->ranges ? launch16<32, false, true, true, true>(a, tpg, (int)total, st) : launch16<32, false, false, true, true>(a, tpg, (int)total, st);
     if (a->b.C == 32) return launch16s<32, false, true>(a, tpg, (int)total, st);
     if (a->xbits) return launch16s<2, true, false>(a, tpg, (int)total, st);
     return launch16s<2, false, false>(a, tpg, (int)total, st);
diff --git a/graph_neural_net_amd/csrc/mlp_bwd_x3.hip b/graph_neural_net_amd/csrc/mlp_bwd_x3.hip
--- a/graph_neural_net_amd/csrc/mlp_bwd_x3.hip
+++ b/graph_neural_net_amd/csrc/mlp_bwd_x3.hip
@@ -529,6 +529,7 @@
 
 extern "C" int fgnn_mlp_bwd_x3(const fgnn_mlp_bwd_args *a, void *stream) {
     FGNN_CHECK(a != nullptr, "fgnn_mlp_bwd_x3: null args");
+    FGNN_CHECK(!a->dy_records, "fgnn_mlp_bwd_x3: dy_records is a form of fgnn_mlp_bwd_t16");
     FGNN_CHECK(a->G > 0 && a->N > 0, "fgnn_mlp_bwd_x3: bad G=%d N=%d", a->G, a->N);
     FGNN_CHECK(mlp_x3_supported(a->a.C, a->b.C, a->depth, 1),
                "fgnn_mlp_bwd_x3: built for depth 3 and 2, 32, 32+2, 32+32 input channels (got depth %d, %d + %d); use fgnn_mlp_bwd",
diff --git a/graph_neural_net_amd/csrc/pool_score.hip b/graph_neural_net_amd/csrc/pool_score.hip
--- a/graph_neural_net_amd/csrc/pool_score.hip
+++ b/graph_neural_net_amd/csrc/pool_score.hip
@@ -281,6 +281,31 @@
     }
 }
 
+__global__ __launch_bounds__(256) void colmax_bwd_rec_kernel(const float *de, const int *idx, const int *nvalid, int GC, int C, int N,
+                                                             float2 *rec, const fgnn_slab y, float *s12) {
+    const int lane = threadIdx.x & 63, wave = threadIdx.x >> 6;
+    const int gc = blockIdx.x * 4 + wave;
+    if (gc >= GC) return;
+    const int g = gc / C, c = gc - g * C;
+    const int nv = nvalid_of(nvalid, g, N);
+    const float *zm = y.ptr + (long long)g * y.gstride + (long long)c * y.ldp;
+    const float mean = y.nrm[(long long)gc * 4];
+    float s1 = 0.f, s2 = 0.f;
+    if (lane < N) {
+        const long long t = (long long)gc * N + lane;
+        const int bi = idx[t];
+        const float d = lane < nv ? de[t] : 0.f;
+        rec[t] = make_float2(d, __int_as_float(bi));
+        if (lane < nv) {
+            s1 += d;
+            s2 += d * (zm[(long long)lane * N + bi] - mean);
+        }
+    }
+    s1 = wave_sum(s1);
+    s2 = wave_sum(s2);
+    if (lane < 2) s12[(long long)gc * 2 + lane] = ((lane ? s2 : s1) + 0.f) + (0.f + 0.f);
+}
+
 DEVI void copy_to_lds256(float *dst, const float *src, int n, int tid) {
     constexpr int U = 8;
     int done = 0;
@@ -371,10 +396,16 @@
 
 constexpr int CSPLIT = 4;
 constexpr int CSPLIT_SMALL = 8;
-template <bool CE, bool STAGE>
+struct ScoreRec {
+    const int *idx;
+    fgnn_slab y;
+    float2 *rec;
+    float *s12;
+};
+template <bool CE, bool STAGE, bool REC = false>
 __global__ __launch_bounds__(256) void score_bwd_kernel(const float *e1, const float *e2, const float *scores,
                                                         const float *lse, const float *dscores, const int *nvalid,
-                                                        const float *gscale, int C, int N, float *de1, float *de2) {
+                                                        const float *gscale, int C, int N, float *de1, float *de2, const ScoreRec R = {}) {
     extern __shared__ __attribute__((aligned(16))) float sm[];
     const int cper = (C + (int)gridDim.y - 1) / (int)gridDim.y;
     const int c0 = blockIdx.y * cper;
@@ -385,6 +416,24 @@
     const int b = blockIdx.x, tid = threadIdx.x;
     const int nv = nvalid_of(nvalid, b, N);
     const float *p1 = e1 + ((long long)b * C + c0) * N, *p2 = e2 + ((long long)b * C + c0) * N;
+    const int lane = tid & 63, wave = tid >> 6;
+    int rbi[2][2] = {};
+    float rz[2][2] = {}, rmean[2][2] = {};
+    if constexpr (REC) {
+#pragma unroll
+        for (int it = 0; it < 2; ++it)
+#pragma unroll
+            for (int s = 0; s < 2; ++s) {
+                const int cw = wave + 4 * it, g = b + s * (int)gridDim.x;
+                if (cw < cn) {
+                    const long long gc = (long long)g * C + c0 + cw;
+                    const int nvg = nvalid_of(nvalid, g, N);
+                    rmean[it][s] = R.y.nrm[gc * 4];
+                    if (lane < N) rbi[it][s] = R.idx[gc * N + lane];
+                    if (lane < nvg) rz[it][s] = R.y.ptr[(long long)g * R.y.gstride + (long long)(c0 + cw) * R.y.ldp + (long long)lane * N + rbi[it][s]];
+                }
+            }
+    }
     for (int e = tid; e < cn * N; e += 256) {
         s1[e] = p1[e];
         s2[e] = p2[e];
@@ -424,6 +473,38 @@
         }
     }
     __syncthreads();
+    if constexpr (REC) {
+#pragma unroll
+        for (int it = 0; it < 2; ++it) {
+            const int c = wave + 4 * it, i = lane;
+            if (c >= cn) break;
+            float a1 = 0.f, a2 = 0.f;
+            if (i < nv) {
+                const float *r2 = s2 + c * N, *r1 = s1 + c * N;
+                for (int jj = 0; jj < nv; ++jj) {
+                    a1 = fmaf(r2[jj], dS[i * ld + jj], a1);
+                    a2 = fmaf(r1[jj], dS[jj * ld + i], a2);
+                }
+            }
+#pragma unroll
+            for (int s = 0; s < 2; ++s) {
+                const int g = b + s * (int)gridDim.x;
+                const long long gc = (long long)g * C + c0 + c;
+                const int nvg = nvalid_of(nvalid, g, N);
+                const float d = i < nvg ? (s ? a2 : a1) : 0.f;
+                float t1 = 0.f, t2 = 0.f;
+                if (i < N) R.rec[gc * N + i] = make_float2(d, __int_as_float(rbi[it][s]));
+                if (i < nvg) {
+                    t1 += d;
+                    t2 += d * (rz[it][s] - rmean[it][s]);
+                }
+                t1 = wave_sum(t1);
+                t2 = wave_sum(t2);
+                if (i < 2) R.s12[gc * 2 + i] = ((i ? t2 : t1) + 0.f) + (0.f + 0.f);
+            }
+        }
+        return;
+    }
     for (int e = tid; e < cn * N; e += 256) {
         const int c = e / N, i = e - c * N;
         float a1 = 0.f, a2 = 0.f;
@@ -617,6 +698,19 @@
     return 0;
 }
 
+extern "C" int fgnn_colmax_bwd_rec(const float *de, const int *idx, const int *nvalid, int G, int C, int N, float *rec,
+                                   const fgnn_slab *y, float *s12, void *stream) {
+    FGNN_CHECK(de && idx && rec && s12 && G > 0 && C > 0 && N > 0, "fgnn_colmax_bwd_rec: bad arguments");
+    FGNN_CHECK(N <= 64, "fgnn_colmax_bwd_rec: built for N <= 64 (one row per lane); use fgnn_colmax_bwd");
+    FGNN_CHECK(y && y->ptr && y->nrm && y->C == C, "fgnn_colmax_bwd_rec: needs the normalised input slab of the pooling");
+    FGNN_CHECK((reinterpret_cast<unsigned long long>(rec) & 7ull) == 0, "fgnn_colmax_bwd_rec: rec must be 8-byte aligned");
+    const int tot = G * C;
+    hipLaunchKernelGGL(colmax_bwd_rec_kernel, dim3((unsigned)((tot + 3) / 4)), dim3(256), 0, (hipStream_t)stream, de, idx, nvalid, tot, C, N,
+                       reinterpret_cast<float2 *>(rec), *y, s12);
+    FGNN_LAUNCH_CHECK();
+    return 0;
+}
+
 static int score_lds_bytes(int C, int N) { return (2 * C * N + 4) * (int)sizeof(float); }
 static int score_bwd_lds_bytes(int C, int N, bool stage, int csplit = CSPLIT) {
     const int cper = (C + csplit - 1) / csplit;
@@ -681,6 +775,22 @@
     return launch_score_bwd<true>(e1, e2, scores, lse, nullptr, nvalid, gscale, B, C, N, de1, de2, (hipStream_t)stream);
 }
 
+extern "C" int fgnn_score_ce_bwd_rec(const float *e1, const float *e2, const float *scores, const float *lse, const int *nvalid,
+                                    const float *gscale, int B, int C, int N, const int *idx, const fgnn_slab *y, float *rec, float *s12,
+                                    void *stream) {
+    FGNN_CHECK(e1 && e2 && scores && lse && gscale && idx && rec && s12 && B > 0, "fgnn_score_ce_bwd_rec: bad arguments");
+    FGNN_CHECK(N <= 64 && C <= 32, "fgnn_score_ce_bwd_rec: built for N <= 64, C <= 32; use fgnn_score_ce_bwd + fgnn_colmax_bwd");
+    FGNN_CHECK(y && y->ptr && y->nrm && y->C == C, "fgnn_score_ce_bwd_rec: needs the normalised input slab of the pooling");
+    FGNN_CHECK((reinterpret_cast<unsigned long long>(rec) & 7ull) == 0, "fgnn_score_ce_bwd_rec: rec must be 8-byte aligned");
+    const int csplit = (long long)B * CSPLIT < 256 ? CSPLIT_SMALL : CSPLIT;
+    const int lds = score_bwd_lds_bytes(C, N, true, csplit);
+    const ScoreRec R = {idx, *y, reinterpret_cast<float2 *>(rec), s12};
+    hipLaunchKernelGGL((score_bwd_kernel<true, true, true>), dim3(B, csplit), dim3(256), lds, (hipStream_t)stream, e1, e2, scores, lse, nullptr,
+                       nvalid, gscale, C, N, nullptr, nullptr, R);
+    FGNN_LAUNCH_CHECK();
+    return 0;
+}
+
 extern "C" int fgnn_score_bwd(const float *e1, const float *e2, const float *dscores, const int *nvalid, int B, int C,
                               int N, float *de1, float *de2, void *stream) {
     FGNN_CHECK(e1 && e2 && dscores && de1 && de2 && B > 0, "fgnn_score_bwd: bad arguments");
diff --git a/graph_neural_net_amd/engine.py b/graph_neural_net_amd/engine.py
--- a/graph_neural_net_amd/engine.py
+++ b/graph_neural_net_amd/engine.py
@@ -159,6 +159,7 @@
         self.decisions = None
         self.layout = layout
         self.G, self.N = G, N
+        self.pool_rec = N <= 64 and layout.num_blocks >= 2 and self._t16_bwd3(32)
         self.P = N * N
         self.ldp = _round_up(self.P, 32)
         self.tpg = _lib.tiles_per_graph(N)
@@ -450,6 +451,7 @@
         keys = [(k, j) for k in range(1, L.num_blocks + 1) for j in (1, 2, 3)]
         self._bwd = {
             'dE': torch.empty(self.G, 32, self.N, **f32),
+            'derec': torch.empty(self.G * 32 * self.N * 2, **f32),
             'dy': [act(), act()],
             'dmult': act(), 'dy1': act(), 'dy2': act(),
             's12': {kj: torch.empty(self.G * 32 * 2, **f32) for kj in keys},
@@ -467,9 +469,10 @@
         _lib.call('fgnn_gn_bwd_coef', _lib.ptr(W['s12'][kj]), _lib.ptr(self.nrm[kj]), self._nv(), self.G, 32, self.N,
                   _lib.ptr(W['coef'][slot]), None, None, _lib.stream_ptr())
 
-    def _mlp_bwd(self, params, k, j, a, b, dy, coef, dxa, dxb, acc_a, acc_b, emit=False, dx_strides=None):
+    def _mlp_bwd(self, params, k, j, a, b, dy, coef, dxa, dxb, acc_a, acc_b, emit=False, dx_strides=None, rec=False):
         args = self._mlp_bwd_args(params, k, j, a, b, dy, coef, dxa, dxb, acc_a, acc_b, emit, dx_strides)
         entry = 'fgnn_mlp_bwd_x3' if (self.x3 and j != 3) else 'fgnn_mlp_bwd'
+        args.dy_records = int(rec)
         if j == 3 and b is not None and self._t16_bwd3(b.C) and _lib.load().fgnn_mlp_bwd_t16_supported(C.byref(args)):
             entry = 'fgnn_mlp_bwd_t16'
         elif self._packs[('b', k, j)][0] == 5:
@@ -538,6 +541,12 @@
         else:
             self._set_gscale(grad_scale / self.total_nodes)
         e1, e2 = self.E[:B], self.E[B:]
+        if self.pool_rec:
+            K = self.layout.num_blocks
+            out = self._slab_z(K, 3, params)
+            _lib.call('fgnn_score_ce_bwd_rec', _lib.ptr(e1), _lib.ptr(e2), _lib.ptr(self.scores), _lib.ptr(self.lse), self._nv(), _lib.ptr(gs_t),
+                      B, 32, N, _lib.ptr(self.idx), C.byref(out), _lib.ptr(W['derec']), _lib.ptr(W['s12'][(K, 3)]), st)
+            return self.backward_from_dE(params, grads, None, finalize=finalize, pooled_rec=True)
         _lib.call('fgnn_score_ce_bwd', _lib.ptr(e1), _lib.ptr(e2), _lib.ptr(self.scores), _lib.ptr(self.lse),
                   self._nv(), _lib.ptr(gs_t), B, 32, N, _lib.ptr(W['dE'][:B]), _lib.ptr(W['dE'][B:]), st)
         return self.backward_from_dE(params, grads, W['dE'], finalize=finalize)
@@ -548,7 +557,7 @@
             W['gscale'].fill_(gs)
             W['gscale_value'] = gs
 
-    def backward_from_dE(self, params, grads, dE, finalize=True, dx=None):
+    def backward_from_dE(self, params, grads, dE, finalize=True, dx=None, pooled_rec=False):
         L = self.layout
         W = self._alloc_bwd()
         st = _lib.stream_ptr()
@@ -557,8 +566,14 @@
         in_prologue = bool(_lib.load().fgnn_mlp_bwd_coef_tiles_supported(self.G, self.N)) and self.ranges is None
         dy = W['dy'][0]
         out = self._slab_z(K, 3, params)
-        _lib.call('fgnn_colmax_bwd', _lib.ptr(dE), _lib.ptr(self.idx), self._nv(), self.G, 32, self.N,
-                  _lib.ptr(dy), gs, self.ldp, C.byref(out), _lib.ptr(W['s12'][(K, 3)]), st)
+        if pooled_rec:
+            dy = W['derec']
+        if pooled_rec and dE is not None:
+            _lib.call('fgnn_colmax_bwd_rec', _lib.ptr(dE), _lib.ptr(self.idx), self._nv(), self.G, 32, self.N,
+                      _lib.ptr(dy), C.byref(out), _lib.ptr(W['s12'][(K, 3)]), st)
+        elif not pooled_rec:
+            _lib.call('fgnn_colmax_bwd', _lib.ptr(dE), _lib.ptr(self.idx), self._nv(), self.G, 32, self.N,
+                      _lib.ptr(dy), gs, self.ldp, C.byref(out), _lib.ptr(W['s12'][(K, 3)]), st)
         for k in range(K, 0, -1):
             sin = self._slab_in(k, params)
             first = (k == 1)
@@ -571,7 +586,8 @@
                                        'and a contiguous (G, c0, N, N) fp32 dx')
                 din, dxs = dx, (L.c0 * self.P, self.P)
             self._mlp_bwd(params, k, 3, self._slab_raw(self.mult[k]), sin, dy,
-                          None if k == K else ('tiles' if in_prologue else W['coef'][2]), W['dmult'], din, False, False, dx_strides=dxs)
+                          None if k == K else ('tiles' if in_prologue else W['coef'][2]), W['dmult'], din, False, False, dx_strides=dxs,
+                          rec=pooled_rec and k == K)
             if first and self.struct1 and self.xbits is not None and dxs is None:
                 self._struct_bwd(params)
                 dy = din
diff --git a/include/fgnn_hip.h b/include/fgnn_hip.h
--- a/include/fgnn_hip.h
+++ b/include/fgnn_hip.h
@@ -178,6 +178,9 @@
 int fgnn_score_ce_bwd(const float *e1, const float *e2, const float *scores, const float *lse,
                       const int *nvalid, const float *gscale, int B, int C, int N,
                       float *de1, float *de2, void *stream);
+int fgnn_score_ce_bwd_rec(const float *e1, const float *e2, const float *scores, const float *lse, const int *nvalid,
+                          const float *gscale, int B, int C, int N, const int *idx, const fgnn_slab *y, float *rec, float *s12,
+                          void *stream);
 
 int fgnn_ce_fwd(const float *scores, const int *nvalid, int B, int N, float *lse, float *pair_loss, void *stream);
 int fgnn_ce_bwd(const float *scores, const float *lse, const int *nvalid, const float *gscale, int B, int N,
@@ -187,6 +190,8 @@
 
 int fgnn_colmax_bwd(const float *de, const int *idx, const int *nvalid, int G, int C, int N,
                     float *dy, long long gstride, long long ldp, const fgnn_slab *y, float *s12, void *stream);
+int fgnn_colmax_bwd_rec(const float *de, const int *idx, const int *nvalid, int G, int C, int N,
+                        float *rec, const fgnn_slab *y, float *s12, void *stream);
 
 int fgnn_gn_bwd_stats(const float *dy, long long dgstride, long long ldd,
                       const float *z, long long zgstride, long long ldz, const float *nrm,
@@ -223,7 +228,11 @@
     const float *xdeg;
     const int *ranges;
     int cu_share;
+    int dy_records;
 } fgnn_mlp_bwd_args;
+#ifdef __cplusplus
+static_assert(sizeof(fgnn_mlp_bwd_args) == 368, "fgnn_mlp_bwd_args is passed by value as a kernel argument: keep its size");
+#endif
 int fgnn_mlp_bwd(const fgnn_mlp_bwd_args *args, void *stream);
 int fgnn_mlp_bwd_x3(const fgnn_mlp_bwd_args *args, void *stream);
 int fgnn_mlp_bwd_pair(const fgnn_mlp_bwd_args *m1, const fgnn_mlp_bwd_args *m2, void *stream);
```
